# ucas-vg/PointTinyBenchmark

Measured on AMD Instinct MI355X. Metric: img/s (640x640) CPR R50-FPN fwd+loss, higher is better.
Workload: dtype fp32

## Files before the change

include/cpr_hip.h:

```cpp
#ifndef CPR_HIP_H
#define CPR_HIP_H
#ifdef __cplusplus
extern "C" {
#endif

#define CPR_ERR_ARG (-1001)
#define CPR_ERR_UNSUPPORTED (-1002)

int cpr_version(void);

#define CPR_CONV_RELU 1
#define CPR_CONV_OUT_BF16 2
#define CPR_CONV_RES_MASK 4
#define CPR_CONV_COLSUM 8
int cpr_conv2d_fwd(const float* in, const float* wgt, float* out, const float* scale, const float* bias,
                   const float* residual, const float* in_a, const float* in_b, float* gn_part, int N, int H, int W,
                   int Cin, int Cout, int KH, int KW, int stride, int pad, int Kpad, int flags, int in_relu,
                   int* variant_out, void* stream);
int cpr_conv2d_fwd_dil(const float* in, const float* wgt, float* out, const float* scale, const float* bias,
                       const float* residual, const float* in_a, const float* in_b, float* gn_part, int N, int H, int W,
                       int Cin, int Cout, int KH, int KW, int stride, int pad, int dil, int Kpad, int flags, int in_relu,
                       int* variant_out, void* stream);

int cpr_conv2d_dual_fwd(const float* in, const float* wgt, const float* in2, const float* wgt2, float* out,
                        const float* scale, const float* bias, const float* scale2, const float* bias2, int N, int H, int W,
                        int Cin, int Cout, int KH, int KW, int stride, int pad, int Kpad, int H2, int W2, int Cin2,
                        int stride2, int Kpad2, int flags, int* variant_out, void* stream);

int cpr_conv1x1_stream_fwd(const float* in, const float* wgt, float* out, const float* scale, const float* bias,
                           const float* residual, long long M, int Cin, int Cout, int flags, void* stream);

int cpr_conv_wgrad_bf16_workspace_s(int N, int H, int W, int Cin, int Cout, int k, int stride, int dy_bf16, int x_bf16);
int cpr_conv_wgrad_bf16_s(const void* dy, int dy_bf16, const void* x, int x_bf16, float* grad, void* ws, int N, int H, int W, int Cin,
                          int Cout, int k, int stride, int accumulate, void* stream);

#define CPR_WINO_IN_B8 1
#define CPR_WINO_OUT_B8 2
int cpr_wino_pack_weights(const float* wgt, float* u, int Cin, int Cout, int Kpad, void* stream);
int cpr_conv3x3_wino_fwd(const float* in, const float* u, float* out, const float* scale, const float* bias,
                         const float* in_a, const float* in_b, float* gn_part, int N, int H, int W, int Cin, int Cout,
                         int flags, int in_relu, int layout, void* stream);
int cpr_wino32_pack_weights(const float* wgt, float* u, int Cin, int Cout, int Kpad, void* stream);
int cpr_conv3x3_wino32_slots(int H, int W);
int cpr_conv3x3_wino32_fwd(const float* in, const float* u, float* out, const float* scale, const float* bias,
                           const float* in_a, const float* in_b, float* gn_part, int N, int H, int W, int Cin, int Cout,
                           int flags, int in_relu, int layout, void* stream);
int cpr_gn_apply_b8(const float* x, const float* a, const float* b, float* y, int N, int H, int W, int C, int relu,
                    void* stream);

int cpr_conv2d_fwd_bf16(const void* in, const void* wgt, const void* wgt_frag, void* out, const float* scale, const float* bias,
                        const void* residual, float* gn_part, int N, int H, int W, int Cin, int Cout, int KH, int KW,
                        int stride, int pad, int Kpad, int relu, int out_fp32, int* variant_out, void* stream);
int cpr_conv2d_bf16_mask_slots(int N, int H, int W, int Cin, int Cout, int KH, int KW, int stride, int pad, int out_fp32);
int cpr_conv2d_dgrad_bf16_fused(const void* in, const void* wgt, const void* wgt_frag, float* out32, void* out16, const float* add32,
                                const void* mask, float* part, int N, int H, int W, int Cin, int Cout, int KH, int KW, int stride,
                                int pad, int Kpad, int* variant_out, void* stream);
int cpr_stem7x7s2_bf16(const float* in, const void* wgt, const float* scale, const float* bias, void* out, int N, int H, int W,
                       int relu, int layout, void* stream);
int cpr_stem7x7s2_pool_bf16(const float* in, const void* wgt, const float* scale, const float* bias, void* out, int N, int H,
                            int W, int layout, void* stream);
int cpr_maxpool3x3s2_bf16(const void* in, void* out, int N, int H, int W, int C, void* stream);
int cpr_gn_stats_bf16(const void* x, float* part, int N, int HW, int C, int P, void* stream);
int cpr_gn_apply_bf16(const void* x, const float* a, const float* b, const void* up, void* y, int N, int H, int W,
                      int C, int UH, int UW, int relu, void* stream);

int cpr_nchw_to_nhwc4(const float* in, float* out, int N, int C, int H, int W, void* stream);
int cpr_nhwc_to_nchw(const float* in, float* out, int N, int C, int H, int W, void* stream);
int cpr_stem7x7s2_pool_f32(const float* in, const float* wgt, const float* scale, const float* bias, float* out, int N, int H,
                           int W, int layout, void* stream);
int cpr_maxpool3x3s2(const float* in, float* out, int N, int H, int W, int C, void* stream);
int cpr_stem_deep_fwd(const float* in, const float* w1, const float* s1, const float* b1, const float* w2, const float* s2,
                      const float* b2, const float* w3, const float* s3, const float* b3, float* mid1, float* mid2, void* out, int N,
                      int H, int W, int layout, int out_bf16, void* stream);
int cpr_stem3x3s2_fwd(const float* in, const float* w, const float* scale, const float* bias, float* out, int N, int H, int W,
                      int layout, void* stream);
int cpr_stem3x3s2_wgrad_workspace(int N, int H, int W);
int cpr_stem3x3s2_wgrad(const float* dy, const float* in, float* gw, float* ws, int N, int H, int W, int layout, void* stream);
int cpr_avgpool_fwd(const void* in, void* out, int N, int H, int W, int C, int s, int bf16, void* stream);
int cpr_avgpool_bwd(const void* g, const void* add, void* dx, int N, int H, int W, int C, int s, int bf16, void* stream);
int cpr_maxpool3x3s2_rec(const float* in, float* out, unsigned char* arg, int N, int H, int W, int C, void* stream);
int cpr_maxpool3x3s2_bf16_rec(const void* in, void* out, unsigned char* arg, int N, int H, int W, int C, void* stream);
int cpr_stem7x7s2_pool_f32_rec(const float* in, const float* wgt, const float* scale, const float* bias, float* out,
                               unsigned char* arg, int N, int H, int W, int layout, void* stream);
int cpr_stem7x7s2_pool_bf16_rec(const float* in, const void* wgt, const float* scale, const float* bias, void* out,
                                unsigned char* arg, int N, int H, int W, int layout, void* stream);
int cpr_stem_pool_bwd_blocks(long long M);
int cpr_stem_pool_bwd(const float* dp, const unsigned char* arg, float* dy, float* part, int N, int OH, int OW, void* stream);
int cpr_stem_wgrad_f32_workspace(int N, int H, int W);
int cpr_stem_wgrad_f32(const float* dy, const float* in, float* gw, float* ws, int N, int H, int W, int layout, void* stream);

int cpr_gn_stats(const float* x, float* part, int N, int HW, int C, int P, void* stream);
int cpr_gn_finalize(const float* part, const float* gamma, const float* beta, float* a_out, float* b_out,
                    float* mean_out, float* rstd_out, int N, int P, int C, int G, int HW, float eps, void* stream);
int cpr_gn_apply(const float* x, const float* a, const float* b, const float* up, float* y, int N, int H, int W,
                 int C, int UH, int UW, int relu, void* stream);

int cpr_box_centers(const float* boxes, float* centers, int n, void* stream);

#define CPR_PROB_SIGMOID 0
#define CPR_PROB_SOFTMAX 1
#define CPR_PROB_NORMED_SIGMOID 2
#define CPR_PROB_IDENTITY 3

int cpr_logit_project(const float* x, const float* w, const float* bias, const float* in_a, const float* in_b,
                      float* out, int N, int HW, int Cin, int J, int in_relu, void* stream);

int cpr_neg_mask_loss(const float* logit, int J, const float* centers, const int* labels, const int* gt_start,
                      const int* pad_hw, unsigned char* mask, double* partial, int N, int H, int W, int C,
                      float stride, float d2_thr, float eps, int class_wise, int prob_type, float norm_p,
                      int mask_classes, int* n_partial, void* stream);

int cpr_bag_sample(const float* map, int J, const float* centers, const int* gt_img, const int* pad_hw,
                   const float* offsets, float* pts, unsigned char* valid, float* out, int G, int K, int H, int W,
                   float stride, int align_corners, const float* pad_value, void* stream);

int cpr_grid_bag(const float* map, int J, const float* points, const int* gt_img, int R, int Kmax, float radius_px,
                 const float* pad_value, float* pts, unsigned char* valid, int* ws_cell, int* count, float* out, int G,
                 int H, int W, float stride, int align_corners, void* stream);

int cpr_mil_loss(const float* logits, int J, int ins_off, const unsigned char* valid, const int* labels,
                 const float* gt_weight, float* bag_ws, const double* neg_partial, int n_partial, int num_bags,
                 int bag_stride, int bag_off, int bag_len, int ctr_off, int ctr_stride, int ctr_count, int ctr_mod,
                 int C, float eps, int prob_type, float norm_p, int binary_ins, int allpos, float w_mil, float w_gt,
                 float w_neg, int neg_from_gt, float* out5, void* stream);

int cpr_refine(const float* logits, int J, const float* pts, const unsigned char* valid, const float* centers, int Rv,
               int ctr_stride, const int* labels, const int* gt_img, const int* gt_start, const int* img_hw,
               const unsigned char* not_refine_in, float* refine_pts, float* scores, unsigned char* not_refine,
               unsigned char* chosen, int G, int Kt, int Kv, int C, int prob_type, float norm_p, float gt_alpha,
               float merge_th, float refine_th, int use_nearest, int use_classify, int score_max, void* stream);

int cpr_point_assign(const float* points, const float* gt_bboxes, int n, int k, float scale, int pos_num,
                     long long* gt_inds, float* ws_best, int* ws_lvl, void* stream);

int cpr_hungarian_cost(const float* pred, int pred_stride, const float* logits, int C, const float* gt,
                       const int* labels, float* costT, int M, int G, float w_cls, float alpha, float gamma,
                       float eps, float w_dis, float fx, float fy, int p_norm, void* stream);
int cpr_match_cost(const float* pred, int pdim, const float* logits, int C, const float* gt, const int* labels, float* costT,
                   int M, int G, const float* terms, int ncls, int nreg, void* stream);

int cpr_lsa_topk(const float* costT, const int* m_of, const int* g_of, const long long* cost_off,
                 const long long* col_off, const long long* row_off, int num_problems, int topk, long long* gt_inds,
                 double* ws_v, double* ws_spc, int* ws_path, int* ws_row4col, unsigned char* ws_sc,
                 unsigned char* ws_active, int* ws_cols, int* ws_remaining, int* ws_pos, double* ws_u,
                 int* ws_col4row, unsigned char* ws_sr, int* status, int max_cols, int max_rows, void* stream);

int cpr_topk_desc(const float* scores, int n, int k, float* out_vals, long long* out_idx, void* stream);

int cpr_nms_candidates(const float* boxes, int box_stride, const float* scores, const float* factors, int n, int C,
                       float score_thr, float* cand_boxes, float* cand_scores, int* cand_labels, long long* cand_inds,
                       int* count, void* stream);
int cpr_nms_workspace(int n);
int cpr_nms(const float* boxes, const float* scores, const int* labels, int n, float iou_thr, long long* keep_idx,
            int* num_keep, int* ws_order, float* ws_boxes, unsigned long long* ws_mask, void* stream);
int cpr_topk_desc_batched(const float* scores, int B, int n, int k, float* out_vals, long long* out_idx, void* stream);
int cpr_nms_candidates_batched(const float* boxes, int box_stride, const float* scores, const float* factors, int B, int n,
                               int C, float score_thr, float* cand_boxes, float* cand_scores, int* cand_labels,
                               long long* cand_inds, int* count, void* stream);
int cpr_nms_batched(const float* boxes, const float* scores, const int* labels, const int* n_dev, int B, int cap,
                    float iou_thr, long long* keep_idx, int* num_keep, int* ws_order, float* ws_boxes,
                    unsigned long long* ws_mask, long long ws_stride, void* stream);

int cpr_p2p_decode(const float* reg, const float* point_anchor, float* pred, float* anchor, int N, int H, int W, int k,
                   float stride, float gamma, void* stream);
int cpr_tap_sum3x3(const float* R, const float* bias, float* out, int N, int H, int W, int J, void* stream);
int cpr_rowmax_sigmoid(const float* logits, float* out, long long M, int C, void* stream);
int cpr_sigmoid(const float* x, float* y, long long n, void* stream);
int cpr_p2p_loss(const float* logits, const float* pred, const long long* gt_inds, const float* gt_pts,
                 const int* gt_labels, const int* gt_start, double* ws_partial, float* out, int B, int M, int C,
                 float alpha, float gamma, float beta, float pos_w, float neg_w, float reg_norm, float w_cls,
                 float w_reg, int cls_mode, int reg_mode, void* stream);

int cpr_conv2d_wgrad_workspace(int N, int OH, int OW, int Cin, int Cout, int KH, int KW);
int cpr_conv2d_wgrad(const float* dy, const float* x, const float* in_a, const float* in_b, float* grad_w, float* ws,
                     int N, int H, int W, int Cin, int Cout, int KH, int KW, int stride, int pad, int in_relu,
                     int accumulate, void* stream);
int cpr_conv2d_wgrad_dil(const float* dy, const float* x, float* grad_w, float* ws, int N, int H, int W, int Cin, int Cout, int KH,
                         int KW, int stride, int pad, int dil, int accumulate, void* stream);
int cpr_conv3x3_wino_wgrad_workspace(int N, int H, int W, int Cin, int Cout);
int cpr_conv3x3_wino_wgrad(const float* dy, const float* x, const float* in_a, const float* in_b, float* grad_w, float* ws,
                           int N, int H, int W, int Cin, int Cout, int in_relu, int accumulate, void* stream);
int cpr_gn_bwd(const float* x, const float* dz, const float* a, const float* b, const float* mean, const float* rstd,
               const float* gamma, float* dx, float* dgamma, float* dbeta, float* ws_part, float* ws_k, int N, int HW,
               int C, int G, int P, int relu, int accumulate, void* stream);
int cpr_gn_bwd_bf16(const void* x_bf16, const float* dz, const float* a, const float* b, const float* mean, const float* rstd,
                    const float* gamma, float* dx, void* dx_bf16, float* dgamma, float* dbeta, float* ws_part, float* ws_k, int N,
                    int HW, int C, int G, int P, int relu, int accumulate, void* stream);
int cpr_gn_bwd_bf16_dz16(const void* x_bf16, const void* dz_bf16, const float* a, const float* b, const float* mean, const float* rstd,
                         const float* gamma, float* dx, void* dx_bf16, float* dgamma, float* dbeta, float* ws_part, float* ws_k,
                         int N, int HW, int C, int G, int P, int relu, int accumulate, void* stream);
int cpr_upsample_add_bwd(const float* dfine, float* dcoarse, int N, int H, int W, int UH, int UW, int C, int accumulate,
                         void* stream);
int cpr_relu_bwd_colsum_ws(long long M, int C);
int cpr_relu_bwd_colsum(const float* dy, const float* add, const void* y, int y_bf16, float* g_out, void* g16_out, float* colsum,
                        float* ws_part, long long M, int C, int accumulate, void* stream);
int cpr_part_colsum(const float* part, float* out, float* ws, int tiles, int C, void* stream);
int cpr_bn_fold_bwd(float* Gw, const float* weight, const float* scale, const float* mean, const float* inv_sigma,
                    const float* colsum_g, float* dgamma, float* dbeta, int Cout, int K, void* stream);
int cpr_bn_fold_bwd_part(float* Gw, const float* weight, const float* scale, const float* mean, const float* inv_sigma, const float* part,
                         int tiles, float* dgamma, float* dbeta, int Cout, int K, void* stream);
int cpr_axpby(float* y, const float* x, float alpha, float beta, long long n, void* stream);
int cpr_phase_scatter_add(const float* src, float* dst, int N, int Hs, int Ws, int C, int H, int W, int py, int px,
                          int sh, int sw, int s, void* stream);
int cpr_zero_insert(const float* dy, float* out, int N, int OH, int OW, int C, int H, int W, int s, void* stream);
int cpr_pack_weights_grouped(const float* w, const float* scale, float* out, int C, int cg, int transpose, void* stream);
int cpr_pack_weights_grouped_multi(const void* jobs_dev, int n, int total_blocks, void* stream);
int cpr_conv_group_fwd(const float* x, const float* wp, float* out, const float* scale, const float* bias, int N, int H, int W, int C,
                       int cg, int stride, int flags, void* stream);
int cpr_conv_group_wgrad_workspace(int N, int OH, int OW, int C, int cg);
int cpr_conv_group_wgrad(const float* dy, const float* x, float* grad_w, float* ws, int N, int H, int W, int C, int cg, int stride,
                         int accumulate, void* stream);
int cpr_conv_group_fwd_pitch(const float* x, const float* wp, float* out, const float* scale, const float* bias, int N, int H, int W,
                             int C, int Cp, int cg, int stride, int flags, void* stream);
int cpr_conv_group_wgrad_pitch(const float* dy, const float* x, float* grad_w, float* ws, int N, int H, int W, int C, int Cp, int cg,
                               int stride, int accumulate, void* stream);
int cpr_conv_group_fwd_dil(const float* x, const float* wp, float* out, const float* scale, const float* bias, int N, int H, int W,
                           int C, int cg, int dil, int flags, void* stream);
int cpr_conv_group_wgrad_dil(const float* dy, const float* x, float* grad_w, float* ws, int N, int H, int W, int C, int cg, int dil,
                             int accumulate, void* stream);
int cpr_res2_pack_weights(const float* w, const float* scale, float* out, int width, int transpose, void* stream);
int cpr_res2_conv_fwd(const float* x, int x_pitch, int x_off, const float* add, int add_pitch, int add_off, const float* wp, float* out,
                      int out_pitch, int out_off, const float* scale, const float* bias, int N, int IH, int IW, int OH, int OW, int width,
                      int stride, int transposed, int flags, void* stream);
int cpr_res2_conv_wgrad_workspace(int N, int OH, int OW, int width);
int cpr_res2_conv_wgrad(const float* dy, int dy_pitch, int dy_off, const float* x, int x_pitch, int x_off, const float* add, int add_pitch,
                        int add_off, float* grad_w, float* ws, int N, int H, int W, int width, int stride, int accumulate, void* stream);
int cpr_res2_relu_bwd_colsum(float* g, int g_pitch, int g_off, const float* carry, int c_pitch, int c_off, const float* y, int y_pitch,
                             int y_off, float* colsum, float* ws, long long M, int width, void* stream);
int cpr_res2_pool_fwd(const float* x, int x_pitch, int x_off, float* out, int out_pitch, int out_off, int N, int H, int W, int width,
                      int stride, void* stream);
int cpr_res2_pool_bwd(const float* dy, int dy_pitch, int dy_off, float* dx, int dx_pitch, int dx_off, int N, int H, int W, int width,
                      int stride, void* stream);
int cpr_splat_chunks(int H, int W, int w);
int cpr_splat_gap(const float* u, float* g, float* ws, int N, int H, int W, int w, void* stream);
int cpr_splat_attn(const float* g, const float* fc1w, const float* fc1b, const float* s1, const float* t1, const float* fc2w,
                   const float* fc2b, float* att, float* z, int N, int w, int inter, void* stream);
int cpr_splat_apply(const float* u, const float* att, float* out, int N, int H, int W, int w, int pool, void* stream);
int cpr_splat_attn_grad(const float* dout, const float* u, float* datt, float* ws, int N, int H, int W, int w, int pool, void* stream);
int cpr_splat_attn_bwd(const float* att, const float* datt, const float* z, const float* g, const float* fc1w, const float* fc1b,
                       const float* s1, const float* mean, const float* inv_sigma, const float* fc2w, float* dg, float* ws, float* gfc1w,
                       float* gfc1b, float* gbnw, float* gbnb, float* gfc2w, float* gfc2b, int N, int w, int inter, void* stream);
int cpr_splat_apply_bwd(const float* dout, const float* u, const float* att, const float* dg, float* du, float* colsum, float* ws, int N,
                        int H, int W, int w, int pool, void* stream);
#define CPR_DW_IN_CLAMP6 1
#define CPR_DW_RELU6 2
int cpr_dw3x3_pack(const float* w, const float* scale, float* wp, int C, void* stream);
int cpr_dw3x3_fwd(const float* x, const float* wp, const float* scale, const float* bias, float* y, int N, int H, int W, int C, int stride,
                  int flags, void* stream);
int cpr_dw3x3_dgrad_workspace(int N, int H, int W, int C);
int cpr_dw3x3_dgrad(const float* dy, const float* wp, const float* add, const float* mask, float* dx, float* colsum, float* ws, int N, int H,
                    int W, int C, int stride, void* stream);
int cpr_dw3x3_wgrad_workspace(int N, int H, int W, int C, int stride);
int cpr_dw3x3_wgrad(const float* dy, const float* x, float* grad_w, float* ws, int N, int H, int W, int C, int stride, int in_clamp6,
                    int accumulate, void* stream);
int cpr_relu6_bwd_colsum_ws(long long M, int C);
int cpr_relu6_bwd_colsum(const float* dy, const float* add, const float* y, float* g_out, float* colsum, float* ws, long long M, int C,
                         void* stream);
int cpr_clamp6(float* x, long long n, void* stream);
int cpr_subsample2(const void* x, int x_bf16, const float* a, const float* b, void* out, int N, int H, int W, int C, void* stream);
int cpr_subsample2_bwd_add(const float* dfine, const float* dcoarse, float* out, int N, int H, int W, int C, void* stream);
int cpr_relu_mask_add(const float* dz, const float* d, const void* y, int y_bf16, float* out, long long n, void* stream);
int cpr_gn_apply2(const float* x1, const float* a1, const float* b1, const float* x2, const float* a2, const float* b2, float* y, int N, int H,
                  int W, int C, void* stream);
int cpr_gn_apply2_bf16(const void* x1, const float* a1, const float* b1, const void* x2, const float* a2, const float* b2, void* y, int N,
                       int H, int W, int C, void* stream);
typedef struct cpr_bfp_level {
    const void* x;
    const float* a;
    const float* b;
    void* y;
    void* arg;
    int H, W;
    float sy, sx;
} cpr_bfp_level;
int cpr_bfp_gather(const cpr_bfp_level* levels, int L, int refine_level, float* bsf, int N, int C, int arg_wide, void* stream);
int cpr_bfp_gather_bf16(const cpr_bfp_level* levels, int L, int refine_level, void* bsf, int N, int C, int arg_wide, void* stream);
int cpr_bfp_scatter(const cpr_bfp_level* levels, int L, int refine_level, const float* ref, const float* ref_a, const float* ref_b, int N,
                    int C, int arg_wide, void* stream);
int cpr_bfp_scatter_bf16(const cpr_bfp_level* levels, int L, int refine_level, const void* ref, const float* ref_a, const float* ref_b,
                         int N, int C, int arg_wide, void* stream);
int cpr_bfp_scatter_bwd(const cpr_bfp_level* levels, int L, int refine_level, float* d_ref, int N, int C, int arg_wide, void* stream);
int cpr_bfp_gather_bwd(const cpr_bfp_level* levels, int L, int refine_level, const float* d_bsf, int N, int C, int arg_wide, void* stream);
typedef struct cpr_hrfpn_level {
    void* p;
    int H, W;
} cpr_hrfpn_level;
int cpr_hrfpn_fuse(const cpr_hrfpn_level* levels, int L, const float* bias, float* out, int N, int C, void* stream);
int cpr_hrfpn_fuse_bf16(const cpr_hrfpn_level* levels, int L, const float* bias, void* out, int N, int C, void* stream);
int cpr_hrfpn_pool(const float* out, int H0, int W0, const cpr_hrfpn_level* levels, int K1, int N, int C, void* stream);
int cpr_hrfpn_pool_bf16(const void* out, int H0, int W0, const cpr_hrfpn_level* levels, int K1, int N, int C, void* stream);
int cpr_hrfpn_pool_bwd_blocks(int N, int H0, int W0);
int cpr_hrfpn_pool_bwd(const cpr_hrfpn_level* gs, int K, float* d_out, float* part, int N, int C, void* stream);
int cpr_hrfpn_fuse_bwd(const float* d_out, int H0, int W0, const cpr_hrfpn_level* dys, int L1, int N, int C, void* stream);
typedef struct cpr_hrnet_term {
    const void* p;
    int k;
} cpr_hrnet_term;
int cpr_hrnet_fuse(const cpr_hrnet_term* terms, int T, float* out, int N, int H, int W, int C, void* stream);
int cpr_hrnet_fuse_bwd_blocks(int N, int H, int W, int C, int K);
int cpr_hrnet_fuse_bwd(const float* dy, const float* y, float* g, float* const* pools, int K, float* part, int N, int H, int W, int C,
                       void* stream);
int cpr_loss_bwd(const float* lmap, const unsigned char* neg_mask, const float* out5, const float* bag_logits,
                 const unsigned char* valid, const int* labels, const float* gt_weight, const float* bag_ws,
                 const float* centers, const int* gt_img, const float* offsets, float* dbag_ws, float* dmap, float* win_ws,
                 int* win_org, int win, int N, int H, int W, int J, int Jd, int ins_off, int G, int K, int C, float stride,
                 float eps, float w_mil, float w_gt, float w_neg, const float* upstream, void* stream);
int cpr_bag_gather_bwd(const float* dsample, int J, const float* centers, const int* gt_img, const float* offsets,
                       float* win_ws, int* win_org, int win, float* dmap, int N, int H, int W, int Jd, int G, int K,
                       float stride, void* stream);
int cpr_bag_points_gather_bwd(const float* dsample, int J, const float* pts, const int* code, const int* gt_img, float* dmap,
                              float* wout_ws, float* dbias, int N, int H, int W, int Jd, int G, int Kt, float stride,
                              int align_corners, void* stream);
int cpr_loss_bwd_general(const float* lmap, const unsigned char* neg_mask, const float* out5, const float* bag_logits,
                         const unsigned char* valid, const int* labels, const float* gt_weight, const float* bag_ws, float* dbag,
                         float* dmap, int N, int H, int W, int J, int Jd, int ins_off, int num_bags, int bag_stride, int bag_off,
                         int bag_len, int ctr_off, int ctr_stride, int ctr_count, int ctr_mod, int C, float eps, int prob_type,
                         float norm_p, int binary_ins, int allpos, float w_mil, float w_gt, float w_neg, int neg_from_gt,
                         const float* upstream, void* stream);
int cpr_pack_weights(const float* w, const float* scale, float* out, int O, int I, int KH, int KW, int colsp, int Kpad,
                     int transpose, void* stream);
int cpr_pack_weights_bf16(const float* w, const float* scale, void* out, void* frag, int O, int I, int KH, int KW, int transpose,
                          void* stream);
int cpr_spin(long long ticks, void* stream);
int cpr_bn_fold(const float* gamma, const float* beta, const float* mean, const float* var, float eps, float* scale,
                float* shift, float* inv_sigma, int C, void* stream);
int cpr_bn_train_ws(long long M, int C);
int cpr_bn_batch_stats(const float* y, const float* gamma, const float* beta, float* running_mean, float* running_var,
                       long long* num_batches_tracked, float momentum, float eps, float* mean, float* rstd, float* scale, float* shift,
                       float* center, float* cmean, float* cshift, float* ws, long long M, int C, void* stream);
int cpr_bn_apply(const float* y, const float* center, const float* scale, const float* shift, const float* residual, const float* y2,
                 const float* center2, const float* scale2, const float* shift2, float* out, long long M, int C, int relu, void* stream);
int cpr_bn_train_bwd(const float* dout, const float* z, const float* y, const float* center, const float* mean, const float* rstd,
                     const float* gamma, float* dy, float* dgamma, float* dbeta, float* ws, long long M, int C, void* stream);
int cpr_bn_sync_ws(long long M, int C);
int cpr_bn_sync_stats_local(const float* y, double* record, float* ws, long long M, int C, void* stream);
int cpr_bn_sync_stats_merge(const double* records, int R, const float* y, const float* gamma, const float* beta, float* running_mean,
                            float* running_var, long long* num_batches_tracked, float momentum, float eps, float* mean, float* rstd,
                            float* scale, float* shift, float* center, float* cmean, float* cshift, double* count, int C, void* stream);
int cpr_bn_sync_bwd_local(const float* dout, const float* z, const float* y, const float* center, const float* mean, const float* rstd,
                          float* dgamma, float* dbeta, double* record, float* ws, long long M, int C, void* stream);
// ... 74 lines not shown
```

pointtinybenchmark_amd/csrc/common.h:

```cpp
#pragma once
#include <hip/hip_runtime.h>
#include <stdint.h>

#define CPR_OK 0
#define CPR_ERR_ARG (-1001)
#define CPR_ERR_UNSUPPORTED (-1002)

#define CPR_CONV_RELU 1
#define CPR_CONV_OUT_BF16 2
#define CPR_CONV_RES_MASK 4
#define CPR_CONV_COLSUM 8

#define CPR_WINO_IN_B8 1
#define CPR_WINO_OUT_B8 2

#define CPR_CHECK_ARG(cond) \
    do {                    \
        if (!(cond)) return CPR_ERR_ARG; \
    } while (0)

#define CPR_LAUNCH_STATUS()                          \
    do {                                             \
        hipError_t e_ = hipGetLastError();           \
        return e_ == hipSuccess ? CPR_OK : -(int)e_; \
    } while (0)

typedef float f32x4 __attribute__((ext_vector_type(4)));
typedef float f32x16 __attribute__((ext_vector_type(16)));

__device__ __forceinline__ float wave_sum(float v) {
#pragma unroll
    for (int o = 32; o > 0; o >>= 1) v += __shfl_xor(v, o, 64);
    return v;
}
__device__ __forceinline__ double wave_sum_d(double v) {
#pragma unroll
    for (int o = 32; o > 0; o >>= 1) v += __shfl_xor(v, o, 64);
    return v;
}
__device__ __forceinline__ float wave_max(float v) {
#pragma unroll
    for (int o = 32; o > 0; o >>= 1) v = fmaxf(v, __shfl_xor(v, o, 64));
    return v;
}
__device__ __forceinline__ float wave_min(float v) {
#pragma unroll
    for (int o = 32; o > 0; o >>= 1) v = fminf(v, __shfl_xor(v, o, 64));
    return v;
}

__device__ __forceinline__ float sleef_expf_u10(float d) {
    const float q = rintf(__fmul_rn(d, 1.442695040888963407359924681001892137426645954152985934135449406931f));
    float s = __fmaf_rn(q, -0.693145751953125f, d);
    s = __fmaf_rn(q, -1.428606765330187045e-06f, s);
    float u = 0.000198527617612853646278381f;
    u = __fmaf_rn(u, s, 0.00139304355252534151077271f);
    u = __fmaf_rn(u, s, 0.00833336077630519866943359f);
    u = __fmaf_rn(u, s, 0.0416664853692054748535156f);
    u = __fmaf_rn(u, s, 0.166666671633720397949219f);
    u = __fmaf_rn(u, s, 0.5f);
    u = __fadd_rn(1.0f, __fmaf_rn(__fmul_rn(s, s), u, s));
    const int qi = (int)q, h = qi >> 1;
    u = __fmul_rn(u, __int_as_float((h + 127) << 23));
    u = __fmul_rn(u, __int_as_float((qi - h + 127) << 23));
    if (d < -104.f) u = 0.f;
    if (d > 104.f) u = INFINITY;
    return u;
}
__device__ __forceinline__ float sigmoid_torch_cpu(float x) { return __fdiv_rn(1.f, __fadd_rn(1.f, sleef_expf_u10(-x))); }

__device__ __forceinline__ float sq_norm(float x, float y) {
    return __fadd_rn(__fmul_rn(x, x), __fmul_rn(y, y));
}
__device__ __forceinline__ float d2_chain(float px, float py, float pn, float cx, float cy, float cn) {
    float acc = __fmul_rn(-2.f * px, cx);
    acc = __fmaf_rn(-2.f * py, cy, acc);
    acc = __fadd_rn(pn, acc);
    acc = __fadd_rn(acc, cn);
    return acc;
}

static inline int cdiv(int a, int b) { return (a + b - 1) / b; }
static inline int cpr_images_per_launch(int N, long long bytes_per_image, int align = 1) {
    const long long lim = (1ll << 31) - 1;
    if (bytes_per_image <= 0 || bytes_per_image > lim) return 0;
    const long long fit = lim / bytes_per_image;
    if (fit >= N) return N;
    const long long launches = (N + fit - 1) / fit;
    long long n = (N + launches - 1) / launches;
    n = (n + align - 1) / align * align;
    if (n > fit) n = fit / align * align;
    return (int)n;
}
static inline long long cpr_max2(long long a, long long b) { return a > b ? a : b; }
static inline long long cdivll(long long a, long long b) { return (a + b - 1) / b; }
```

pointtinybenchmark_amd/csrc/conv_wino.hip:

```cpp
#include <type_traits>
#include "common.h"

typedef float f32x2 __attribute__((ext_vector_type(2)));
typedef int i32x4 __attribute__((ext_vector_type(4)));
typedef float f32x2 __attribute__((ext_vector_type(2)));

__device__ __forceinline__ f32x2 pk_add(f32x2 a, f32x2 b) {
    f32x2 r; asm("v_pk_add_f32 %0, %1, %2" : "=v"(r) : "v"(a), "v"(b)); return r;
}
__device__ __forceinline__ f32x2 pk_sub(f32x2 a, f32x2 b) {
    f32x2 r; asm("v_pk_add_f32 %0, %1, %2 neg_lo:[0,1] neg_hi:[0,1]" : "=v"(r) : "v"(a), "v"(b)); return r;
}
__device__ __forceinline__ f32x2 pk_col01(f32x2 t01, f32x2 t23) {
    f32x2 r; asm("v_pk_add_f32 %0, %1, %2 op_sel:[0,0] op_sel_hi:[1,0] neg_lo:[0,1] neg_hi:[0,0]" : "=v"(r) : "v"(t01), "v"(t23)); return r;
}
__device__ __forceinline__ f32x2 pk_col23(f32x2 t01, f32x2 t23) {
    f32x2 r; asm("v_pk_add_f32 %0, %1, %2 op_sel:[1,0] op_sel_hi:[1,1] neg_lo:[1,0] neg_hi:[0,1]" : "=v"(r) : "v"(t01), "v"(t23)); return r;
}
__device__ __forceinline__ f32x2 pk_fma(f32x2 a, f32x2 b, f32x2 c) {
    f32x2 r; asm("v_pk_fma_f32 %0, %1, %2, %3" : "=v"(r) : "v"(a), "v"(b), "v"(c)); return r;
}

struct WinoParams {
    const float* in;
    const float* u;
    float* out;
    const float* scale;
    const float* bias;
    float* gn_part;
    const float* in_a;
    const float* in_b;
    int in_relu, out_b8;
    int N, H, W, Cin, Cout, relu, RY, RX, regions, tilesN, nch;
    int tpx;
};

constexpr int WBUF = 16 * 64 * 8;

__global__ void wino_pack_kernel(const float* __restrict__ w, float* __restrict__ u, int Cin, int Cout, int Kpad) {
    const int idx = blockIdx.x * blockDim.x + threadIdx.x;
    if (idx >= Cin * Cout) return;
    const int ci = idx % Cin, co = idx / Cin;
    float g[3][3];
#pragma unroll
    for (int a = 0; a < 3; ++a)
#pragma unroll
        for (int b = 0; b < 3; ++b) g[a][b] = w[(size_t)co * Kpad + (a * 3 + b) * Cin + ci];
    float t[4][3];
#pragma unroll
    for (int b = 0; b < 3; ++b) {
        t[0][b] = g[0][b];
        t[1][b] = 0.5f * (g[0][b] + g[1][b] + g[2][b]);
        t[2][b] = 0.5f * (g[0][b] - g[1][b] + g[2][b]);
        t[3][b] = g[2][b];
    }
    const int tn = co >> 6, cl = co & 63, chunk = ci >> 3, k = ci & 7, nch = Cin >> 3;
    float* dst = u + ((size_t)(tn * nch + chunk) * 16) * 512 + cl * 8 + 4 * ((k >> 2) ^ ((cl >> 3) & 1)) + (k & 3);
#pragma unroll
    for (int i = 0; i < 4; ++i) {
        dst[(i * 4 + 0) * 512] = t[i][0];
        dst[(i * 4 + 1) * 512] = 0.5f * (t[i][0] + t[i][1] + t[i][2]);
        dst[(i * 4 + 2) * 512] = 0.5f * (t[i][0] - t[i][1] + t[i][2]);
        dst[(i * 4 + 3) * 512] = t[i][2];
    }
}

template <int ABL, bool INB8, bool XF, int TSPREAD = 1, int VAR = 0>
__global__ __launch_bounds__(512, 1) void conv_wino_kernel(WinoParams p) {
    constexpr bool DEEP = (VAR & 1) != 0, UDMA = (VAR & 4) != 0, USINGLE = (VAR & 2) != 0 && !UDMA;
    constexpr int XFMAX = 512;
    constexpr int RAWROW = 148;
    constexpr int RAWBUF = 18 * RAWROW;
    __shared__ __attribute__((aligned(16))) float smem[4 * WBUF + 2 * RAWBUF + (XF ? 4 * XFMAX : 0)];
    float* Vs = smem;
    float* Us = smem + 2 * WBUF;

    const int tid = threadIdx.x, lane = tid & 63;
    const int wave = __builtin_amdgcn_readfirstlane(tid >> 6);
    const int wi = wave & 3;
    const int nh = wave >> 2;

    const int pixbytes = INB8 ? 32 : p.Cin * 4;
    const int chunk_bytes = INB8 ? p.H * p.W * 32 : 32;
    const __amdgpu_buffer_rsrc_t rs_in = __builtin_amdgcn_make_buffer_rsrc(
        const_cast<float*>(p.in), 0, (int)((size_t)p.N * p.H * p.W * p.Cin * 4), 0x00020000);
    const __amdgpu_buffer_rsrc_t rs_u = __builtin_amdgcn_make_buffer_rsrc(
        const_cast<float*>(p.u), 0, (int)((size_t)p.tilesN * p.nch * WBUF * 4), 0x00020000);
    float* Rw = smem + 4 * WBUF;
    float* ABs = smem + 4 * WBUF + 2 * RAWBUF;
    int par = 0;
    int upyx[2], raw_wr[2];
#pragma unroll
    for (int k = 0; k < 2; ++k) {
        const int pix = (tid + 512 * k) >> 1;
        const int py = pix / 18, px = pix - py * 18;
        upyx[k] = py << 8 | px;
        raw_wr[k] = py * RAWROW + px * 8 + (tid & 1) * 4;
    }
    const bool second_unit = wave < 3;
    const bool unit1_live = tid + 512 < 648;
    const int lch = tid & 7, tyl = (tid >> 3) & 7, ltile = wave * 8 + tyl;
    const float* t_rd = Rw + (2 * tyl) * RAWROW + (2 * wave) * 8 + lch;
    const int v_wr = ltile * 8 + 4 * ((lch >> 2) ^ ((ltile >> 3) & 1)) + (lch & 3);
    const int last = p.nch - 1;
    const float relu_floor = (XF && p.in_relu) ? 0.f : -INFINITY;

    struct Tile {
        int rg, tn, n, oy0, ox0, n0;
        int voffA[2];
        unsigned uok;
        bool any_pad, valid;
    };
    const int T = p.regions * p.tilesN;
    const int per = (T + 7) >> 3;
    const int ngrp = p.tpx > 0 ? p.tilesN / p.tpx : 1;
    const int per_r = p.tpx > 0 ? (p.regions * ngrp + 7) / 8 : 0;
    auto setup = [&](int vb) {
        Tile t;
        if (p.tpx > 0) {
            const int x = vb & 7, s = vb >> 3;
            const int sr = s / p.tpx;
            t.rg = (x / ngrp) * per_r + sr;
            t.tn = (x % ngrp) * p.tpx + (s - sr * p.tpx);
            t.valid = sr < per_r && t.rg < p.regions;
            if (!t.valid) { t.rg = 0; t.tn = 0; }
        } else {
            const int tile = (vb & 7) * per + (vb >> 3);
            t.valid = vb < per * 8 && tile < T;
            const int tl = t.valid ? tile : 0;
            t.rg = tl / p.tilesN; t.tn = tl - t.rg * p.tilesN;
        }
        t.n = t.rg / (p.RY * p.RX);
        const int rrem = t.rg - t.n * p.RY * p.RX;
        const int ry = rrem / p.RX, rx = rrem - ry * p.RX;
        t.oy0 = ry * 16; t.ox0 = rx * 16; t.n0 = t.tn * 64;
        const int img_base = INB8 ? (t.n * (p.Cin >> 3)) * p.H * p.W * 32 : t.n * p.H * p.W * p.Cin * 4;
        t.uok = 0;
#pragma unroll
        for (int k = 0; k < 2; ++k) {
            const int iy = t.oy0 - 1 + (upyx[k] >> 8), ix = t.ox0 - 1 + (upyx[k] & 255);
            const bool ok = (k == 0 || unit1_live) & ((unsigned)iy < (unsigned)p.H) & ((unsigned)ix < (unsigned)p.W);
            t.uok |= (ok ? 1u : 0u) << k;
            t.voffA[k] = ok ? img_base + (iy * p.W + ix) * pixbytes + (tid & 1) * 16 : (int)0x80000000;
        }
        t.any_pad = XF && __builtin_amdgcn_ballot_w64(t.uok != (unit1_live ? 3u : 1u)) != 0;
        return t;
    };

    f32x4 sp[2][2];
    f32x4 su[(USINGLE || UDMA) ? 1 : 2][4];
    float tab_a = 0.f, tab_b = 0.f;
    f32x2 d[4][2];
    if (ABL & 9) { sp[0][0] = f32x4{1.f, 1.f, 1.f, 1.f}; sp[0][1] = sp[0][0]; sp[1][0] = sp[0][0]; sp[1][1] = sp[0][0]; }
    Tile cur = setup(blockIdx.x);
    auto ld_a = [&](const Tile& t, int ck, int k) {
        return __builtin_bit_cast(f32x4, __builtin_amdgcn_raw_buffer_load_b128(rs_in, t.voffA[k], ck * chunk_bytes, 0));
    };
    auto ld_u = [&](const Tile& t, int ck, int z) {
        return __builtin_bit_cast(
            f32x4, __builtin_amdgcn_raw_buffer_load_b128(rs_u, tid * 16 + z * 8192, (t.tn * p.nch + ck) * (WBUF * 4), 0));
    };
    auto prefetch = [&](const Tile& t) {
        if (!(ABL & 8)) {
            sp[0][0] = ld_a(t, 0, 0); sp[1][0] = ld_a(t, 1, 0);
            if (second_unit) { sp[0][1] = ld_a(t, 0, 1); sp[1][1] = ld_a(t, 1, 1); }
        }
        if (!UDMA) {
#pragma unroll
            for (int z = 0; z < 4; ++z) { su[0][z] = ld_u(t, 0, z); if (!USINGLE) su[USINGLE ? 0 : 1][z] = ld_u(t, 1, z); }
        }
        if (XF) {
            if (tid < p.Cin) { tab_a = p.in_a[t.n * p.Cin + tid]; tab_b = p.in_b[t.n * p.Cin + tid]; }
        }
    };
    auto g_a = [&](auto set_c, int chunk, int k) {
        constexpr int SET = decltype(set_c)::value;
        if (ABL & 8) return;
        const int ck = chunk < last ? chunk : last;
        if (k == 0 || second_unit) sp[SET][k] = ld_a(cur, ck, k);
    };
    auto g_u = [&](auto set_c, int chunk, int z) {
        constexpr int SET = (USINGLE || UDMA) ? 0 : decltype(set_c)::value;
        if (!UDMA) su[SET][z] = ld_u(cur, chunk < last ? chunk : last, z);
    };
    const int lds_u0 = (int)(unsigned)(size_t)(smem + 2 * WBUF);
    const size_t u_addr = (size_t)p.u;
    const i32x4 rs_u_raw = {(int)(unsigned)u_addr, (int)(unsigned)(u_addr >> 32) & 0xffff,
                            (int)((size_t)p.tilesN * p.nch * WBUF * 4), 0x00020000};
    auto dma_u = [&](int chunk, int buf, int z) {
        const int soff = (cur.tn * p.nch + chunk) * (WBUF * 4);
        const int m0v = lds_u0 + buf * (WBUF * 4) + z * 8192 + wave * 1024;
        asm volatile("s_nop 4\n\ts_mov_b32 m0, %0\n\ts_nop 0\n\tbuffer_load_dwordx4 %1, %2, %3 offen offset:0 lds"
                     :: "s"(m0v), "v"(tid * 16 + z * 8192), "s"(rs_u_raw), "s"(soff) : "memory");
    };
    auto dma_wait = [&](auto npatch_c) {
        constexpr int NP = decltype(npatch_c)::value;
        if (NP == 0) asm volatile("s_waitcnt vmcnt(0)" ::: "memory");
        else if (second_unit) asm volatile("s_waitcnt vmcnt(%0)" :: "n"(2 * NP) : "memory");
        else asm volatile("s_waitcnt vmcnt(%0)" :: "n"(NP) : "memory");
    };
    auto affine = [&](f32x4 v, f32x4 a4, f32x4 b4, int k) {
        if (ABL & 64) v = v * a4 + b4;
        else {
            const f32x2 lo = pk_fma(f32x2{v.x, v.y}, f32x2{a4.x, a4.y}, f32x2{b4.x, b4.y});
            const f32x2 hi = pk_fma(f32x2{v.z, v.w}, f32x2{a4.z, a4.w}, f32x2{b4.z, b4.w});
            v = f32x4{lo.x, lo.y, hi.x, hi.y};
        }
        v.x = fmaxf(v.x, relu_floor); v.y = fmaxf(v.y, relu_floor); v.z = fmaxf(v.z, relu_floor); v.w = fmaxf(v.w, relu_floor);
        if (cur.any_pad) {
            asm volatile("");
            if (!((cur.uok >> k) & 1u)) v = f32x4{0.f, 0.f, 0.f, 0.f};
        }
        return v;
    };
    f32x4 xa4, xb4;
    auto xf_fetch = [&](int chunk) {
        const float* tab = ABs + par * 2 * XFMAX + (chunk < last ? chunk : last) * 8 + (tid & 1) * 4;
        xa4 = *reinterpret_cast<const f32x4*>(tab);
        xb4 = *reinterpret_cast<const f32x4*>(tab + XFMAX);
    };
    auto r_a = [&](auto set_c, int buf, int k) {
        constexpr int SET = decltype(set_c)::value;
        if (k == 1 && !second_unit) return;
        f32x4 v = sp[SET][k];
        if (XF) v = affine(v, xa4, xb4, k);
        if (k == 0 || unit1_live) *reinterpret_cast<f32x4*>(Rw + buf * RAWBUF + raw_wr[k]) = v;
    };
    auto r_a_pro = [&](int chunk01, int k) {
        if (k == 1 && !second_unit) return;
        f32x4 v = chunk01 ? sp[1][k] : sp[0][k];
        if (XF) {
            const float* tab = ABs + par * 2 * XFMAX + chunk01 * 8 + (tid & 1) * 4;
            v = affine(v, *reinterpret_cast<const f32x4*>(tab), *reinterpret_cast<const f32x4*>(tab + XFMAX), k);
        }
        if (k == 0 || unit1_live) *reinterpret_cast<f32x4*>(Rw + chunk01 * RAWBUF + raw_wr[k]) = v;
    };
    auto r_u = [&](auto set_c, int buf, int z) {
        constexpr int SET = (USINGLE || UDMA) ? 0 : decltype(set_c)::value;
        if (!UDMA) *reinterpret_cast<f32x4*>(Us + buf * WBUF + tid * 4 + z * 2048) = su[SET][z];
    };
    auto t_read = [&](int buf, int r) {
#pragma unroll
        for (int s = 0; s < 2; ++s)
            d[r][s] = f32x2{t_rd[buf * RAWBUF + r * RAWROW + (2 * s) * 8], t_rd[buf * RAWBUF + r * RAWROW + (2 * s + 1) * 8]};
    };
    auto t_row = [&](int buf, int i) {
        float* dst = Vs + buf * WBUF + (i * 4) * 512 + v_wr;
        if (ABL & 64) {
            float ts[4];
#pragma unroll
            for (int s = 0; s < 4; ++s) {
                const float d0 = d[0][s >> 1][s & 1], d1 = d[1][s >> 1][s & 1], d2 = d[2][s >> 1][s & 1], d3 = d[3][s >> 1][s & 1];
                ts[s] = i == 0 ? d0 - d2 : i == 1 ? d1 + d2 : i == 2 ? d2 - d1 : d1 - d3;
            }
            dst[0 * 512] = ts[0] - ts[2];
            dst[1 * 512] = ts[1] + ts[2];
            dst[2 * 512] = ts[2] - ts[1];
            dst[3 * 512] = ts[1] - ts[3];
            return;
        }
        f32x2 t[2];
#pragma unroll
        for (int s = 0; s < 2; ++s)
            t[s] = i == 0 ? pk_sub(d[0][s], d[2][s]) : i == 1 ? pk_add(d[1][s], d[2][s]) : i == 2 ? pk_sub(d[2][s], d[1][s])
                                                                                                  : pk_sub(d[1][s], d[3][s]);
        const f32x2 o01 = pk_col01(t[0], t[1]), o23 = pk_col23(t[0], t[1]);
        dst[0 * 512] = o01.x;
        dst[1 * 512] = o01.y;
        dst[2 * 512] = o23.x;
        dst[3 * 512] = o23.y;
    };
    const int l31 = lane & 31, half = lane >> 5;
    const float* a_lds = Vs + (wi * 4 * 64 + l31) * 8 + 4 * (half ^ ((l31 >> 3) & 1));
    const float* b_lds = Us + (wi * 4 * 64 + nh * 32 + l31) * 8 + 4 * (half ^ ((l31 >> 3) & 1));
    using Set0 = std::integral_constant<int, 0>;
    using Set1 = std::integral_constant<int, 1>;

    if (cur.valid) prefetch(cur);
    if (XF) {
        if (tid < p.Cin) { ABs[tid] = tab_a; ABs[XFMAX + tid] = tab_b; }
        __syncthreads();
    }
    for (int vb = blockIdx.x; cur.valid; vb += gridDim.x) {
    const int rg = cur.rg, n = cur.n, oy0 = cur.oy0, ox0 = cur.ox0, n0 = cur.n0;

    f32x16 acc[4][2];
#pragma unroll
    for (int j = 0; j < 4; ++j)
#pragma unroll
        for (int tb = 0; tb < 2; ++tb)
#pragma unroll
            for (int r = 0; r < 16; ++r) acc[j][tb][r] = 0.f;

    f32x4 fa0[2], fb0, fa1[2], fb1;
#define WFRAG(FA, FB, buf, j, z)                                                                                    \
    do {                                                                                                            \
        if ((z) < 2) FA[(z) < 2 ? (z) : 0] = *reinterpret_cast<const f32x4*>(a_lds + (buf) * WBUF + (j) * 512 + ((z) < 2 ? (z) : 0) * 256); \
        else FB = *reinterpret_cast<const f32x4*>(b_lds + (buf) * WBUF + (j) * 512);                                \
    } while (0)
#define WMFMA(FA, FB, j, q) \
    acc[j][(q) & 1] = __builtin_amdgcn_mfma_f32_32x32x2f32(FA[(q) & 1][(q) >> 1], FB[(q) >> 1], acc[j][(q) & 1], 0, 0, 0)
    r_a_pro(0, 0); r_a_pro(0, 1);
    r_a_pro(1, 0); r_a_pro(1, 1);
    if (UDMA) {
#pragma unroll
        for (int z = 0; z < 4; ++z) dma_u(0, 0, z);
#pragma unroll
        for (int z = 0; z < 4; ++z) dma_u(1, 1, z);
    }
#pragma unroll
    for (int z = 0; z < 4; ++z) r_u(Set0{}, 0, z);
    g_a(Set0{}, 2, 0); g_a(Set0{}, 2, 1);
    if (DEEP) { g_a(Set1{}, 3, 0); g_a(Set1{}, 3, 1); }
#pragma unroll
    for (int z = 0; z < 4; ++z) g_u(Set0{}, USINGLE ? 1 : 2, z);
    __syncthreads();
#pragma unroll
    for (int r = 0; r < 4; ++r) t_read(0, r);
#pragma unroll
    for (int i = 0; i < 4; ++i) t_row(0, i);
    if (TSPREAD == 1) {
#pragma unroll
        for (int r = 0; r < 4; ++r) t_read(1, r);
    }
    if (UDMA) dma_wait(std::integral_constant<int, DEEP ? 2 : 1>{});
    __syncthreads();
#pragma unroll
    for (int z = 0; z < 3; ++z) WFRAG(fa0, fb0, 0, 0, z);

    auto iteration = [&](auto nxt_c, int c) {
        const int buf = c & 1;
        const std::integral_constant<int, DEEP ? 1 - decltype(nxt_c)::value : 0> pset_c{};
#pragma unroll
        for (int q = 0; q < 8; ++q) {
            WMFMA(fa0, fb0, 0, q);
            if (q < 3 && !(ABL & 2)) WFRAG(fa1, fb1, buf, 1, q);
            if (!(ABL & 1)) {
                if (TSPREAD == 0 || TSPREAD == 2) { if (q >= 4) t_read(buf ^ 1, q - 4); }
                else { if (q == 3) t_row(buf ^ 1, 0); if (q == 6) t_row(buf ^ 1, 1); }
            }
            __builtin_amdgcn_sched_barrier(0);
        }
#pragma unroll
        for (int q = 0; q < 8; ++q) {
            WMFMA(fa1, fb1, 1, q);
            if (q < 3 && !(ABL & 2)) WFRAG(fa0, fb0, buf, 2, q);
            if (!(ABL & 1)) {
                if (q & 1) r_u(nxt_c, buf ^ 1, q >> 1);
                else if (TSPREAD == 0) t_row(buf ^ 1, q >> 1);
                else if (TSPREAD == 2) {
                    if (q == 0) {
#pragma unroll
                        for (int i = 0; i < 4; ++i) t_row(buf ^ 1, i);
                    }
                }
                else if (q == 2) t_row(buf ^ 1, 2);
                else if (q == 6) t_row(buf ^ 1, 3);
                if (XF && q == 7) xf_fetch(c + 2);
            }
            __builtin_amdgcn_sched_barrier(0);
        }
#pragma unroll
        for (int q = 0; q < 8; ++q) {
            WMFMA(fa0, fb0, 2, q);
            if (q < 3 && !(ABL & 2)) WFRAG(fa1, fb1, buf, 3, q);
            if (!(ABL & 1)) {
                if (q == 3) { r_a(pset_c, buf, 0); if (TSPREAD == 2) r_a(pset_c, buf, 1); }
                if (q == 4 && TSPREAD != 2) r_a(pset_c, buf, 1);
                if (q == 5 || q == 6 || q == 7) g_u(nxt_c, c + (USINGLE ? 2 : 3), q - 5);
            }
            __builtin_amdgcn_sched_barrier(0);
        }
        asm volatile("" ::: "memory");
        if (UDMA) dma_wait(std::integral_constant<int, DEEP ? 1 : 0>{});
        __builtin_amdgcn_s_waitcnt(0xc07f);
        if (!(ABL & 4)) __builtin_amdgcn_s_barrier();
        asm volatile("" ::: "memory");
        __builtin_amdgcn_sched_barrier(0);
#pragma unroll
        for (int q = 0; q < 8; ++q) {
            WMFMA(fa1, fb1, 3, q);
            if (q < 3 && !(ABL & 2)) WFRAG(fa0, fb0, buf ^ 1, 0, q);
            if (!(ABL & 1)) {
                if (UDMA) {
                    if (q < 4 && c + 2 < p.nch) dma_u(c + 2, buf, q);
                    if (q == 4) g_a(pset_c, c + (DEEP ? 4 : 3), 0);
                    if (q == 6) g_a(pset_c, c + (DEEP ? 4 : 3), 1);
                } else {
                    if (q == 3) g_a(pset_c, c + (DEEP ? 4 : 3), 0);
                    if (q == 5) g_a(pset_c, c + (DEEP ? 4 : 3), 1);
                    if (q == 7) g_u(nxt_c, c + (USINGLE ? 2 : 3), 3);
                }
                if (TSPREAD == 1 && q >= 4) t_read(buf, q - 4);
            }
            __builtin_amdgcn_sched_barrier(0);
        }
    };
    for (int c = 0; c < p.nch; c += 2) {
        iteration(Set1{}, c);
        iteration(Set0{}, c + 1);
    }
#undef WFRAG
#undef WMFMA

    if (ABL & 32) {
        asm volatile("" ::"v"(acc[0][0]), "v"(acc[0][1]), "v"(acc[1][0]), "v"(acc[1][1]));
        asm volatile("" ::"v"(acc[2][0]), "v"(acc[2][1]), "v"(acc[3][0]), "v"(acc[3][1]));
        cur = setup(vb + gridDim.x);
        if (cur.valid) prefetch(cur);
        if (XF && tid < p.Cin) { ABs[(par ^ 1) * 2 * XFMAX + tid] = tab_a; ABs[(par ^ 1) * 2 * XFMAX + XFMAX + tid] = tab_b; }
        par ^= 1;
        __syncthreads();
        continue;
    }
    const Tile nxt = setup(vb + gridDim.x);
    if (nxt.valid) prefetch(nxt);
    __syncthreads();
    float* Rs = smem;
#pragma unroll
    for (int tb = 0; tb < 2; ++tb)
#pragma unroll
        for (int r = 0; r < 16; ++r) {
            const int trow = tb * 32 + (r & 3) + 8 * (r >> 2) + 4 * half;
            const float m0 = acc[0][tb][r], m1 = acc[1][tb][r], m2 = acc[2][tb][r], m3 = acc[3][tb][r];
            Rs[((wi * 2 + 0) * 64 + trow) * 64 + nh * 32 + l31] = m0 + m1 + m2;
            Rs[((wi * 2 + 1) * 64 + trow) * 64 + nh * 32 + l31] = m1 - m2 - m3;
        }
    __syncthreads();
    const int c4 = tid & 15;
    const int co = n0 + c4 * 4;
    f32x4 sc = {1.f, 1.f, 1.f, 1.f}, bi = {0.f, 0.f, 0.f, 0.f};
    if (p.scale) sc = *reinterpret_cast<const f32x4*>(p.scale + co);
    if (p.bias) bi = *reinterpret_cast<const f32x4*>(p.bias + co);
    const __amdgpu_buffer_rsrc_t rs_out = __builtin_amdgcn_make_buffer_rsrc(
        p.out, 0, (int)((size_t)p.N * p.H * p.W * p.Cout * 4), 0x00020000);
    f32x4 gs = {0.f, 0.f, 0.f, 0.f}, gq = {0.f, 0.f, 0.f, 0.f};
#pragma unroll
    for (int k = 0; k < 2; ++k) {
        const int t = (tid >> 4) + 32 * k;
        const int oy = oy0 + 2 * (t & 7), ox = ox0 + 2 * (t >> 3);
#pragma unroll
        for (int b = 0; b < 2; ++b) {
            const f32x4 r0 = *reinterpret_cast<const f32x4*>(Rs + ((0 * 2 + b) * 64 + t) * 64 + c4 * 4);
            const f32x4 r1 = *reinterpret_cast<const f32x4*>(Rs + ((1 * 2 + b) * 64 + t) * 64 + c4 * 4);
            const f32x4 r2 = *reinterpret_cast<const f32x4*>(Rs + ((2 * 2 + b) * 64 + t) * 64 + c4 * 4);
            const f32x4 r3 = *reinterpret_cast<const f32x4*>(Rs + ((3 * 2 + b) * 64 + t) * 64 + c4 * 4);
            f32x4 y[2] = {r0 + r1 + r2, r1 - r2 - r3};
#pragma unroll
            for (int a = 0; a < 2; ++a) {
                f32x4 v = y[a] * sc + bi;
                if (p.relu) { v.x = fmaxf(v.x, 0.f); v.y = fmaxf(v.y, 0.f); v.z = fmaxf(v.z, 0.f); v.w = fmaxf(v.w, 0.f); }
                const bool ok = (oy + a < p.H) & (ox + b < p.W);
                const unsigned off = !ok ? 0x80000000u
                    : p.out_b8 ? (unsigned)((((n * (p.Cout >> 3) + (co >> 3)) * p.H + oy + a) * p.W + ox + b) * 8 + (co & 7)) * 4u
                               : (unsigned)(((n * p.H + oy + a) * p.W + ox + b) * p.Cout + co) * 4u;
                if (!(ABL & 16)) __builtin_amdgcn_raw_buffer_store_b128(__builtin_bit_cast(__attribute__((ext_vector_type(4))) unsigned, v), rs_out, (int)off, 0, 0);
                if (p.gn_part && ok) { gs += v; gq += v * v; }
            }
        }
    }
    if (p.gn_part) {
#pragma unroll
        for (int e = 0; e < 4; ++e) {
            gs[e] += __shfl_xor(gs[e], 16, 64); gs[e] += __shfl_xor(gs[e], 32, 64);
            gq[e] += __shfl_xor(gq[e], 16, 64); gq[e] += __shfl_xor(gq[e], 32, 64);
        }
        __syncthreads();
        if (lane < 16) {
#pragma unroll
            for (int e = 0; e < 4; ++e) {
                smem[(wave * 64 + c4 * 4 + e) * 2 + 0] = gs[e];
                smem[(wave * 64 + c4 * 4 + e) * 2 + 1] = gq[e];
            }
        }
        __syncthreads();
        if (tid < 64) {
            float s = 0.f, q = 0.f;
#pragma unroll
            for (int w8 = 0; w8 < 8; ++w8) { s += smem[(w8 * 64 + tid) * 2]; q += smem[(w8 * 64 + tid) * 2 + 1]; }
            float* dst = p.gn_part + ((size_t)rg * p.Cout + n0 + tid) * 2;
            dst[0] = s; dst[1] = q;
        }
    }
    if (XF && tid < p.Cin) {
        ABs[(par ^ 1) * 2 * XFMAX + tid] = tab_a;
        ABs[(par ^ 1) * 2 * XFMAX + XFMAX + tid] = tab_b;
    }
    par ^= 1;
    __syncthreads();
    cur = nxt;
    }
}

#ifdef CPR_BENCH_HOOKS
static int wino_sched = 0, wino_ablate = 0, wino_var = -1, wino_tpx = -1;
extern "C" int cpr_wino_set_variant(int sched, int ablate) {
    CPR_CHECK_ARG(sched >= 0 && sched <= 2 && ablate >= 0 && ablate <= 64);
    wino_sched = sched;
    wino_ablate = ablate;
    return CPR_OK;
}
extern "C" int cpr_wino_set_staging(int var, int tpx) {
    CPR_CHECK_ARG(var >= -1 && var <= 5 && tpx >= -1 && tpx <= 2);
    wino_var = var;
    wino_tpx = tpx;
    return CPR_OK;
}
#else
constexpr int wino_sched = 0, wino_ablate = 0, wino_var = -1, wino_tpx = -1;
#endif
constexpr int WINO_VAR_DEFAULT = 4, WINO_TPX_DEFAULT = 0;
extern "C" int cpr_wino_pack_weights(const float* wgt, float* u, int Cin, int Cout, int Kpad, hipStream_t stream) {
    CPR_CHECK_ARG(wgt && u && Cin > 0 && Cout > 0 && Cin % 8 == 0 && Cout % 64 == 0 && Kpad >= 9 * Cin);
    hipLaunchKernelGGL(wino_pack_kernel, dim3(cdiv(Cin * Cout, 256)), dim3(256), 0, stream, wgt, u, Cin, Cout, Kpad);
    CPR_LAUNCH_STATUS();
}
static int wino_fwd_launch(const float* in, const float* u, float* out, const float* scale, const float* bias,
                           const float* in_a, const float* in_b, float* gn_part, int N, int H, int W, int Cin,
                           int Cout, int flags, int in_relu, int layout, hipStream_t stream) {
    CPR_CHECK_ARG(in && u && out && N > 0 && H > 0 && W > 0);
    CPR_CHECK_ARG(Cin > 0 && Cout > 0 && Cin % 16 == 0 && Cout % 64 == 0 && Cin >= 32);
    CPR_CHECK_ARG((flags & ~CPR_CONV_RELU) == 0 && (layout & ~3) == 0);
    if (in_a) CPR_CHECK_ARG(in_b && Cin <= 512);
    if ((long long)N * H * W * Cin * 4 >= (1ll << 31) || (long long)N * H * W * Cout * 4 >= (1ll << 31)) return CPR_ERR_UNSUPPORTED;
    WinoParams p;
    p.in = in; p.u = u; p.out = out; p.scale = scale; p.bias = bias; p.gn_part = gn_part;
    p.in_a = in_a; p.in_b = in_b; p.in_relu = in_relu; p.out_b8 = (layout & CPR_WINO_OUT_B8) ? 1 : 0;
    p.N = N; p.H = H; p.W = W; p.Cin = Cin; p.Cout = Cout; p.relu = flags & CPR_CONV_RELU;
    p.RY = (H + 15) / 16; p.RX = (W + 15) / 16;
    p.regions = N * p.RY * p.RX; p.tilesN = Cout / 64; p.nch = Cin / 8;
    const long long T = (long long)p.regions * p.tilesN;
    if (T >= (1ll << 30)) return CPR_ERR_UNSUPPORTED;
    static int cu_of_device[64] = {};
    int dev = 0, ncu = 256;
    if (hipGetDevice(&dev) == hipSuccess && dev >= 0 && dev < 64) {
        if (cu_of_device[dev] == 0) {
            int v = 0;
            if (hipDeviceGetAttribute(&v, hipDeviceAttributeMultiprocessorCount, dev) == hipSuccess && v > 0) cu_of_device[dev] = v;
        }
        if (cu_of_device[dev] > 0) ncu = cu_of_device[dev];
    }
    ncu = (ncu + 7) / 8 * 8;
    int grid = (int)((T + 7) / 8 * 8);
    if (grid > ncu) grid = ncu;
    const bool b8 = (layout & CPR_WINO_IN_B8) != 0, xf = in_a != nullptr;
    p.tpx = wino_tpx >= 0 ? wino_tpx : WINO_TPX_DEFAULT;
    if (p.tpx > 0 && !(p.tilesN % p.tpx == 0 && 8 % (p.tilesN / p.tpx) == 0)) p.tpx = 0;
    if (p.tpx > 0) {
        const long long per_r = ((long long)p.regions * (p.tilesN / p.tpx) + 7) / 8;
        const long long vbs = 8 * per_r * p.tpx;
        if (vbs < grid) grid = (int)vbs;
    }
    const int var = wino_var >= 0 ? wino_var : WINO_VAR_DEFAULT;
#define WLAUNCHV(A_, F_, V_)                                                                                                      \
    do {                                                                                                                         \
        constexpr int TX_ = F_ == 2 ? 2 : 0 ^ F_, TP_ = F_ == 2 ? 2 : 1 ^ F_;                                                     \
        if (b8 && xf) hipLaunchKernelGGL((conv_wino_kernel<A_, true, true, TX_, V_>), dim3(grid), dim3(512), 0, stream, p);       \
        else if (b8) hipLaunchKernelGGL((conv_wino_kernel<A_, true, false, TP_, V_>), dim3(grid), dim3(512), 0, stream, p);       \
        else if (xf) hipLaunchKernelGGL((conv_wino_kernel<A_, false, true, TX_, V_>), dim3(grid), dim3(512), 0, stream, p);       \
        else hipLaunchKernelGGL((conv_wino_kernel<A_, false, false, TP_, V_>), dim3(grid), dim3(512), 0, stream, p);              \
    } while (0)
#define WLAUNCH(A_, F_) WLAUNCHV(A_, F_, WINO_VAR_DEFAULT)
#ifdef CPR_BENCH_HOOKS
    if ((var != WINO_VAR_DEFAULT || wino_sched == 2) && !wino_ablate) {
        switch (var * 3 + wino_sched) {
            case 0: WLAUNCHV(0, 0, 0); break;
            case 1: WLAUNCHV(0, 1, 0); break;
            case 2: WLAUNCHV(0, 2, 0); break;
            case 6: WLAUNCHV(0, 0, 2); break;
            case 7: WLAUNCHV(0, 1, 2); break;
            case 8: WLAUNCHV(0, 2, 2); break;
            case 9: WLAUNCHV(0, 0, 3); break;
            case 10: WLAUNCHV(0, 1, 3); break;
            case 11: WLAUNCHV(0, 2, 3); break;
            case 12: WLAUNCHV(0, 0, 4); break;
            case 13: WLAUNCHV(0, 1, 4); break;
            case 14: WLAUNCHV(0, 2, 4); break;
            default: return CPR_ERR_UNSUPPORTED;
        }
    } else if (wino_ablate || wino_sched) {
        switch (wino_ablate) {
            case 0: WLAUNCH(0, 1); break;
            case 1: WLAUNCH(1, 0); break;
            case 2: WLAUNCH(2, 0); break;
            case 4: WLAUNCH(4, 0); break;
            case 8: WLAUNCH(8, 0); break;
            case 16: WLAUNCH(16, 0); break;
            case 32: WLAUNCH(32, 0); break;
            case 64: WLAUNCH(64, 0); break;
            default: WLAUNCH(7, 0); break;
        }
    } else
#endif
    WLAUNCH(0, 0);
#undef WLAUNCH
#undef WLAUNCHV
    CPR_LAUNCH_STATUS();
}

extern "C" int cpr_conv3x3_wino_fwd(const float* in, const float* u, float* out, const float* scale, const float* bias,
                                    const float* in_a, const float* in_b, float* gn_part, int N, int H, int W, int Cin,
                                    int Cout, int flags, int in_relu, int layout, hipStream_t stream) {
    CPR_CHECK_ARG(N > 0 && H > 0 && W > 0 && Cin > 0 && Cout > 0);
    const int per = cpr_images_per_launch(N, (long long)H * W * cpr_max2(Cin, Cout) * 4);
    if (per <= 0) return CPR_ERR_UNSUPPORTED;
    const size_t slots = (size_t)((H + 15) / 16) * ((W + 15) / 16);
    for (int n0 = 0; n0 < N; n0 += per) {
        const int n = N - n0 < per ? N - n0 : per;
        const int rc = wino_fwd_launch(in + (size_t)n0 * H * W * Cin, u, out + (size_t)n0 * H * W * Cout, scale, bias,
                                       in_a ? in_a + (size_t)n0 * Cin : nullptr, in_b ? in_b + (size_t)n0 * Cin : nullptr,
                                       gn_part ? gn_part + (size_t)n0 * slots * Cout * 2 : nullptr, n, H, W, Cin, Cout, flags,
                                       in_relu, layout, stream);
        if (rc != CPR_OK) return rc;
    }
    return CPR_OK;
}
```

pointtinybenchmark_amd/csrc/conv_wino32.hip:

```cpp
#include "common.h"

typedef float f32x2 __attribute__((ext_vector_type(2)));
typedef int i32x4 __attribute__((ext_vector_type(4)));

struct Wino32Params {
    const float* in;
    const float* u;
    float* out;
    const float* scale;
    const float* bias;
    float* gn_part;
    const float* in_a;
    const float* in_b;
    int in_relu, in_b8, out_b8;
    int N, H, W, Cin, Cout, relu, RY, RX, regions, tilesN, nch;
    int stagger;
};

constexpr int W32_V = 16 * 32 * 4;
constexpr int W32_U = 16 * 64 * 4;
constexpr int W32_RAW = 192 * 4;
constexpr int W32_XFMAX = 256;
constexpr int W32_LDS = 2 * W32_V + 3 * W32_U + 4 * W32_RAW + 2 * W32_XFMAX;

__global__ void wino32_pack_kernel(const float* __restrict__ w, float* __restrict__ u, int Cin, int Cout, int Kpad) {
    const int idx = blockIdx.x * blockDim.x + threadIdx.x;
    if (idx >= Cin * Cout) return;
    const int ci = idx % Cin, co = idx / Cin;
    float g[3][3];
#pragma unroll
    for (int a = 0; a < 3; ++a)
#pragma unroll
        for (int b = 0; b < 3; ++b) g[a][b] = w[(size_t)co * Kpad + (a * 3 + b) * Cin + ci];
    float t[4][3];
#pragma unroll
    for (int b = 0; b < 3; ++b) {
        t[0][b] = g[0][b];
        t[1][b] = 0.5f * (g[0][b] + g[1][b] + g[2][b]);
        t[2][b] = 0.5f * (g[0][b] - g[1][b] + g[2][b]);
        t[3][b] = g[2][b];
    }
    const int tn = co >> 6, cl = co & 63, chunk = ci >> 2, k = ci & 3, nch = Cin >> 2;
    float* dst = u + ((size_t)(tn * nch + chunk) * 16) * 256 + cl * 4 + k;
#pragma unroll
    for (int i = 0; i < 4; ++i) {
        dst[(i * 4 + 0) * 256] = t[i][0];
        dst[(i * 4 + 1) * 256] = 0.5f * (t[i][0] + t[i][1] + t[i][2]);
        dst[(i * 4 + 2) * 256] = 0.5f * (t[i][0] - t[i][1] + t[i][2]);
        dst[(i * 4 + 3) * 256] = t[i][2];
    }
}

template <bool XF, int ABL = 0>
__global__ __launch_bounds__(256, 2) void conv_wino32_kernel(Wino32Params p) {
    __shared__ __attribute__((aligned(16))) float smem[W32_LDS];
    float* Vs = smem;
    float* Us = smem + 2 * W32_V;
    float* Rw = smem + 2 * W32_V + 3 * W32_U;
    float* ABs = Rw + 4 * W32_RAW;

    const int tid = threadIdx.x, lane = tid & 63;
    const int wave = __builtin_amdgcn_readfirstlane(tid >> 6);
    const int l31 = lane & 31, half = lane >> 5;

    const size_t in_addr = (size_t)p.in, u_addr = (size_t)p.u;
    const i32x4 rs_in = {(int)(unsigned)in_addr, (int)(unsigned)(in_addr >> 32) & 0xffff,
                         (int)((size_t)p.N * p.H * p.W * p.Cin * 4), 0x00020000};
    const i32x4 rs_u = {(int)(unsigned)u_addr, (int)(unsigned)(u_addr >> 32) & 0xffff,
                        (int)((size_t)p.tilesN * p.nch * W32_U * 4), 0x00020000};
    const int lds_u0 = (int)(unsigned)(size_t)Us, lds_raw0 = (int)(unsigned)(size_t)Rw;
    const int pixbytes = p.in_b8 ? 32 : p.Cin * 4;
    const int upy = tid / 18, upx = tid - upy * 18;
    const bool unit_live = tid < 180;
    const int tch = lane & 3, ttx = (lane >> 2) & 7;
    const int t_rd = (2 * wave + half) * 72 + (2 * ttx) * 4 + tch;
    const int t_wrA = ((half ? 12 : 0) * 32 + wave * 8 + ttx) * 4 + tch;
    const int t_wrB = ((half ? 8 : 4) * 32 + wave * 8 + ttx) * 4 + tch;
    const int a_rd = (wave * 4 * 32 + l31) * 4 + 2 * half;
    const int b_rd = (wave * 4 * 64 + l31) * 4 + 2 * half;

    const int T = p.regions * p.tilesN;
    const int per = (T + 7) >> 3;
    const float relu_floor = (XF && p.in_relu) ? 0.f : -INFINITY;

    if ((int)blockIdx.x >= (int)(gridDim.x >> 1)) {
        for (int s = 0; s < p.stagger; ++s) __builtin_amdgcn_s_sleep(127);
    }

    int cur_n = -1;
    for (int vb = blockIdx.x;; vb += gridDim.x) {
        const int tile = (vb & 7) * per + (vb >> 3);
        if (!(vb < per * 8 && tile < T)) break;
        const int rg = tile / p.tilesN, tn = tile - rg * p.tilesN;
        const int n = rg / (p.RY * p.RX);
        const int rrem = rg - n * p.RY * p.RX;
        const int ry = rrem / p.RX, rx = rrem - ry * p.RX;
        const int oy0 = ry * 8, ox0 = rx * 16, n0 = tn * 64;
        const int iy = oy0 - 1 + upy, ix = ox0 - 1 + upx;
        const bool uok = unit_live & ((unsigned)iy < (unsigned)p.H) & ((unsigned)ix < (unsigned)p.W);
        const int img_base = p.in_b8 ? (n * (p.Cin >> 3)) * p.H * p.W * 32 : n * p.H * p.W * p.Cin * 4;
        const int voff_a = uok ? img_base + (iy * p.W + ix) * pixbytes : (int)0x80000000;

        auto dma_u = [&](int chunk, int slot) {
            if (ABL & 2) return;
            const int ck = chunk < p.nch ? chunk : p.nch - 1;
            const int soff = (tn * p.nch + ck) * (W32_U * 4);
#pragma unroll
            for (int z = 0; z < 4; ++z) {
                const int piece = (z * 4 + wave) * 1024;
                const int m0v = lds_u0 + slot * (W32_U * 4) + piece;
                asm volatile("s_nop 4\n\ts_mov_b32 m0, %0\n\ts_nop 0\n\tbuffer_load_dwordx4 %1, %2, %3 offen offset:0 lds"
                             :: "s"(m0v), "v"(piece + lane * 16), "s"(rs_u), "s"(soff) : "memory");
            }
        };
        auto dma_a = [&](int chunk, int slot) {
            if ((ABL & 2) || wave >= 3) return;
            const int ck = chunk < p.nch ? chunk : p.nch - 1;
            const int soff = p.in_b8 ? (ck >> 1) * (p.H * p.W * 32) + (ck & 1) * 16 : ck * 16;
            const int m0v = lds_raw0 + slot * (W32_RAW * 4) + wave * 1024;
            asm volatile("s_nop 4\n\ts_mov_b32 m0, %0\n\ts_nop 0\n\tbuffer_load_dwordx4 %1, %2, %3 offen offset:0 lds"
                         :: "s"(m0v), "v"(voff_a), "s"(rs_in), "s"(soff) : "memory");
        };
        auto wait_older_than_this_chunk = [&]() {
            if (ABL & 2) return;
            if (wave < 3) asm volatile("s_waitcnt vmcnt(5)" ::: "memory");
            else asm volatile("s_waitcnt vmcnt(4)" ::: "memory");
        };
        auto affine_pass = [&](int chunk, int slot) {
            if (!XF || (ABL & 1)) return;
            if (unit_live) {
                const int ck = chunk < p.nch ? chunk : p.nch - 1;
                float* q = Rw + slot * W32_RAW + tid * 4;
                f32x4 v = *reinterpret_cast<const f32x4*>(q);
                const f32x4 a4 = *reinterpret_cast<const f32x4*>(ABs + ck * 4);
                const f32x4 b4 = *reinterpret_cast<const f32x4*>(ABs + W32_XFMAX + ck * 4);
                v = v * a4 + b4;
                v.x = fmaxf(v.x, relu_floor); v.y = fmaxf(v.y, relu_floor); v.z = fmaxf(v.z, relu_floor); v.w = fmaxf(v.w, relu_floor);
                if (!uok) v = f32x4{0.f, 0.f, 0.f, 0.f};
                *reinterpret_cast<f32x4*>(q) = v;
            }
        };
        float e[3][4] = {};
        auto t_read = [&](int slot, int r) {
            if (ABL & 1) return;
#pragma unroll
            for (int s = 0; s < 4; ++s) e[r][s] = Rw[slot * W32_RAW + t_rd + r * 72 + s * 4];
        };
        auto t_write = [&](int buf) {
            if (ABL & 1) return;
            float* dA = Vs + buf * W32_V + t_wrA;
            float* dB = Vs + buf * W32_V + t_wrB;
            float ta[4], tb[4];
#pragma unroll
            for (int s = 0; s < 4; ++s) {
                ta[s] = e[0][s] - e[2][s];
                tb[s] = e[1][s] + (half ? -e[0][s] : e[2][s]);
            }
            dA[0 * 128] = ta[0] - ta[2]; dA[1 * 128] = ta[1] + ta[2]; dA[2 * 128] = ta[2] - ta[1]; dA[3 * 128] = ta[1] - ta[3];
            dB[0 * 128] = tb[0] - tb[2]; dB[1 * 128] = tb[1] + tb[2]; dB[2 * 128] = tb[2] - tb[1]; dB[3 * 128] = tb[1] - tb[3];
        };

        if (XF && n != cur_n) {
            for (int c = tid; c < p.Cin; c += 256) { ABs[c] = p.in_a[n * p.Cin + c]; ABs[W32_XFMAX + c] = p.in_b[n * p.Cin + c]; }
            cur_n = n;
        }
        dma_u(0, 0); dma_u(1, 1);
        dma_a(0, 0); dma_a(1, 1); dma_a(2, 2); dma_a(3, 3);
        asm volatile("s_waitcnt vmcnt(0)" ::: "memory");
        __syncthreads();
        affine_pass(0, 0); affine_pass(1, 1);
        if (XF) __syncthreads();
#pragma unroll
        for (int r = 0; r < 3; ++r) t_read(0, r);
        t_write(0);
        __syncthreads();

        f32x16 acc[4][2];
#pragma unroll
        for (int j = 0; j < 4; ++j)
#pragma unroll
            for (int nb = 0; nb < 2; ++nb)
#pragma unroll
                for (int r = 0; r < 16; ++r) acc[j][nb][r] = 0.f;

        for (int c = 0; c < p.nch; ++c) {
            const int b = c & 1;
            const int uslot = c % 3;
            dma_u(c + 2, (c + 2) % 3);
            dma_a(c + 4, c & 3);
            const float* va = Vs + b * W32_V + a_rd;
            const float* ub = Us + uslot * W32_U + b_rd;
            f32x2 fa[2], fb[2][2];
            fa[0] = *reinterpret_cast<const f32x2*>(va);
            fb[0][0] = *reinterpret_cast<const f32x2*>(ub);
            fb[0][1] = *reinterpret_cast<const f32x2*>(ub + 128);
#pragma unroll
            for (int j = 0; j < 4; ++j) {
                const int cu = j & 1, nx = cu ^ 1;
                acc[j][0] = __builtin_amdgcn_mfma_f32_32x32x2f32(fa[cu].x, fb[cu][0].x, acc[j][0], 0, 0, 0);
                if (j < 3 && !(ABL & 8)) {
                    fa[nx] = *reinterpret_cast<const f32x2*>(va + (j + 1) * 128);
                    fb[nx][0] = *reinterpret_cast<const f32x2*>(ub + (j + 1) * 256);
                    fb[nx][1] = *reinterpret_cast<const f32x2*>(ub + (j + 1) * 256 + 128);
                }
                __builtin_amdgcn_sched_barrier(0);
                acc[j][1] = __builtin_amdgcn_mfma_f32_32x32x2f32(fa[cu].x, fb[cu][1].x, acc[j][1], 0, 0, 0);
                if (j == 0) { t_read((c + 1) & 3, 0); }
                if (j == 1) { t_read((c + 1) & 3, 1); }
                if (j == 2) { t_read((c + 1) & 3, 2); }
                __builtin_amdgcn_sched_barrier(0);
                acc[j][0] = __builtin_amdgcn_mfma_f32_32x32x2f32(fa[cu].y, fb[cu][0].y, acc[j][0], 0, 0, 0);
                if (j == 1) affine_pass(c + 2, (c + 2) & 3);
                __builtin_amdgcn_sched_barrier(0);
                acc[j][1] = __builtin_amdgcn_mfma_f32_32x32x2f32(fa[cu].y, fb[cu][1].y, acc[j][1], 0, 0, 0);
                if (j == 3) t_write(b ^ 1);
                __builtin_amdgcn_sched_barrier(0);
            }
            asm volatile("" ::: "memory");
            wait_older_than_this_chunk();
            __builtin_amdgcn_s_waitcnt(0xc07f);
            if (!(ABL & 4)) __builtin_amdgcn_s_barrier();
            asm volatile("" ::: "memory");
        }
        asm volatile("s_waitcnt vmcnt(0)" ::: "memory");
        __syncthreads();

        float* Rs = smem;
#pragma unroll
        for (int nb = 0; nb < 2; ++nb)
#pragma unroll
            for (int r = 0; r < 16; ++r) {
                const int trow = (r & 3) + 8 * (r >> 2) + 4 * half;
                const float m0 = acc[0][nb][r], m1 = acc[1][nb][r], m2 = acc[2][nb][r], m3 = acc[3][nb][r];
                Rs[((wave * 2 + 0) * 32 + trow) * 64 + nb * 32 + l31] = m0 + m1 + m2;
                Rs[((wave * 2 + 1) * 32 + trow) * 64 + nb * 32 + l31] = m1 - m2 - m3;
            }
        __syncthreads();
        const int c4 = tid & 15;
        const int co = n0 + c4 * 4;
        f32x4 sc = {1.f, 1.f, 1.f, 1.f}, bi = {0.f, 0.f, 0.f, 0.f};
        if (p.scale) sc = *reinterpret_cast<const f32x4*>(p.scale + co);
        if (p.bias) bi = *reinterpret_cast<const f32x4*>(p.bias + co);
        const __amdgpu_buffer_rsrc_t rs_out = __builtin_amdgcn_make_buffer_rsrc(
            p.out, 0, (int)((size_t)p.N * p.H * p.W * p.Cout * 4), 0x00020000);
        f32x4 gs = {0.f, 0.f, 0.f, 0.f}, gq = {0.f, 0.f, 0.f, 0.f};
#pragma unroll
        for (int k = 0; k < 4; ++k) {
            const int it = (tid >> 4) + 16 * k;
            const int t = it & 31, bq = it >> 5;
            const int oy = oy0 + 2 * (t >> 3), ox = ox0 + 2 * (t & 7) + bq;
            const f32x4 r0 = *reinterpret_cast<const f32x4*>(Rs + ((0 * 2 + bq) * 32 + t) * 64 + c4 * 4);
            const f32x4 r1 = *reinterpret_cast<const f32x4*>(Rs + ((1 * 2 + bq) * 32 + t) * 64 + c4 * 4);
            const f32x4 r2 = *reinterpret_cast<const f32x4*>(Rs + ((2 * 2 + bq) * 32 + t) * 64 + c4 * 4);
            const f32x4 r3 = *reinterpret_cast<const f32x4*>(Rs + ((3 * 2 + bq) * 32 + t) * 64 + c4 * 4);
            f32x4 y[2] = {r0 + r1 + r2, r1 - r2 - r3};
#pragma unroll
            for (int a = 0; a < 2; ++a) {
                f32x4 v = y[a] * sc + bi;
                if (p.relu) { v.x = fmaxf(v.x, 0.f); v.y = fmaxf(v.y, 0.f); v.z = fmaxf(v.z, 0.f); v.w = fmaxf(v.w, 0.f); }
                const bool ok = (oy + a < p.H) & (ox < p.W);
                const unsigned off = !ok ? 0x80000000u
                    : p.out_b8 ? (unsigned)((((n * (p.Cout >> 3) + (co >> 3)) * p.H + oy + a) * p.W + ox) * 8 + (co & 7)) * 4u
                               : (unsigned)(((n * p.H + oy + a) * p.W + ox) * p.Cout + co) * 4u;
                __builtin_amdgcn_raw_buffer_store_b128(__builtin_bit_cast(__attribute__((ext_vector_type(4))) unsigned, v), rs_out, (int)off, 0, 0);
                if (p.gn_part && ok) { gs += v; gq += v * v; }
            }
        }
        if (p.gn_part) {
#pragma unroll
            for (int q = 0; q < 4; ++q) {
                gs[q] += __shfl_xor(gs[q], 16, 64); gs[q] += __shfl_xor(gs[q], 32, 64);
                gq[q] += __shfl_xor(gq[q], 16, 64); gq[q] += __shfl_xor(gq[q], 32, 64);
            }
            __syncthreads();
            if (lane < 16) {
#pragma unroll
                for (int q = 0; q < 4; ++q) {
                    smem[(wave * 64 + c4 * 4 + q) * 2 + 0] = gs[q];
                    smem[(wave * 64 + c4 * 4 + q) * 2 + 1] = gq[q];
                }
            }
            __syncthreads();
            if (tid < 64) {
                float s = 0.f, q = 0.f;
#pragma unroll
                for (int w4 = 0; w4 < 4; ++w4) { s += smem[(w4 * 64 + tid) * 2]; q += smem[(w4 * 64 + tid) * 2 + 1]; }
                float* dst = p.gn_part + ((size_t)rg * p.Cout + n0 + tid) * 2;
                dst[0] = s; dst[1] = q;
            }
        }
        __syncthreads();
    }
}

#ifdef CPR_BENCH_HOOKS
static int w32_ablate = 0, w32_wg_per_cu = 2, w32_stagger_pct = 100;
extern "C" int cpr_wino32_set_debug(int ablate, int wg_per_cu, int stagger_pct) {
    CPR_CHECK_ARG(ablate >= 0 && ablate <= 15 && wg_per_cu >= 1 && wg_per_cu <= 2 && stagger_pct >= 0 && stagger_pct <= 400);
    w32_ablate = ablate; w32_wg_per_cu = wg_per_cu; w32_stagger_pct = stagger_pct;
    return CPR_OK;
}
#else
constexpr int w32_ablate = 0, w32_wg_per_cu = 2, w32_stagger_pct = 100;
#endif
extern "C" int cpr_wino32_pack_weights(const float* wgt, float* u, int Cin, int Cout, int Kpad, hipStream_t stream) {
    CPR_CHECK_ARG(wgt && u && Cin > 0 && Cout > 0 && Cin % 4 == 0 && Cout % 64 == 0 && Kpad >= 9 * Cin);
    hipLaunchKernelGGL(wino32_pack_kernel, dim3(cdiv(Cin * Cout, 256)), dim3(256), 0, stream, wgt, u, Cin, Cout, Kpad);
    CPR_LAUNCH_STATUS();
}

extern "C" int cpr_conv3x3_wino32_slots(int H, int W) { return H > 0 && W > 0 ? ((H + 7) / 8) * ((W + 15) / 16) : CPR_ERR_ARG; }

static int wino32_fwd_launch(const float* in, const float* u, float* out, const float* scale, const float* bias,
                             const float* in_a, const float* in_b, float* gn_part, int N, int H, int W, int Cin,
                             int Cout, int flags, int in_relu, int layout, hipStream_t stream) {
    CPR_CHECK_ARG(in && u && out && N > 0 && H > 0 && W > 0);
    CPR_CHECK_ARG(Cin > 0 && Cout > 0 && Cin % 8 == 0 && Cout % 64 == 0 && Cin >= 16);
    CPR_CHECK_ARG((flags & ~CPR_CONV_RELU) == 0 && (layout & ~3) == 0);
    if (in_a) CPR_CHECK_ARG(in_b && Cin <= W32_XFMAX);
    if ((long long)N * H * W * Cin * 4 >= (1ll << 31) || (long long)N * H * W * Cout * 4 >= (1ll << 31)) return CPR_ERR_UNSUPPORTED;
    Wino32Params p;
    p.in = in; p.u = u; p.out = out; p.scale = scale; p.bias = bias; p.gn_part = gn_part;
    p.in_a = in_a; p.in_b = in_b; p.in_relu = in_relu;
    p.in_b8 = (layout & CPR_WINO_IN_B8) ? 1 : 0; p.out_b8 = (layout & CPR_WINO_OUT_B8) ? 1 : 0;
    p.N = N; p.H = H; p.W = W; p.Cin = Cin; p.Cout = Cout; p.relu = flags & CPR_CONV_RELU;
    p.RY = (H + 7) / 8; p.RX = (W + 15) / 16;
    p.regions = N * p.RY * p.RX; p.tilesN = Cout / 64; p.nch = Cin / 4;
    const long long T = (long long)p.regions * p.tilesN;
    if (T >= (1ll << 30)) return CPR_ERR_UNSUPPORTED;
    static int cu_of_device[64] = {};
    int dev = 0, ncu = 256;
    if (hipGetDevice(&dev) == hipSuccess && dev >= 0 && dev < 64) {
        if (cu_of_device[dev] == 0) {
            int v = 0;
            if (hipDeviceGetAttribute(&v, hipDeviceAttributeMultiprocessorCount, dev) == hipSuccess && v > 0) cu_of_device[dev] = v;
        }
        if (cu_of_device[dev] > 0) ncu = cu_of_device[dev];
    }
    ncu = (ncu + 7) / 8 * 8;
    int grid = (int)((T + 7) / 8 * 8);
    if (grid > w32_wg_per_cu * ncu) grid = w32_wg_per_cu * ncu;
    p.stagger = grid > ncu ? (int)(((long long)p.nch * 16 * 65 * w32_stagger_pct / 100 + 8127) / 8128) : 0;
#ifdef CPR_BENCH_HOOKS
#define W32L(A_)                                                                                                      \
    do {                                                                                                              \
        if (in_a) hipLaunchKernelGGL((conv_wino32_kernel<true, A_>), dim3(grid), dim3(256), 0, stream, p);           \
        else hipLaunchKernelGGL((conv_wino32_kernel<false, A_>), dim3(grid), dim3(256), 0, stream, p);               \
    } while (0)
    switch (w32_ablate) {
        case 0: W32L(0); break;
        case 1: W32L(1); break;
        case 2: W32L(2); break;
        case 3: W32L(3); break;
        case 4: W32L(4); break;
        case 7: W32L(7); break;
        case 8: W32L(8); break;
        case 15: W32L(15); break;
        default: return CPR_ERR_UNSUPPORTED;
    }
#undef W32L
#else
    if (in_a) hipLaunchKernelGGL((conv_wino32_kernel<true>), dim3(grid), dim3(256), 0, stream, p);
    else hipLaunchKernelGGL((conv_wino32_kernel<false>), dim3(grid), dim3(256), 0, stream, p);
#endif
    CPR_LAUNCH_STATUS();
}

extern "C" int cpr_conv3x3_wino32_fwd(const float* in, const float* u, float* out, const float* scale, const float* bias,
                                      const float* in_a, const float* in_b, float* gn_part, int N, int H, int W, int Cin,
                                      int Cout, int flags, int in_relu, int layout, hipStream_t stream) {
    CPR_CHECK_ARG(N > 0 && H > 0 && W > 0 && Cin > 0 && Cout > 0);
    const int per = cpr_images_per_launch(N, (long long)H * W * cpr_max2(Cin, Cout) * 4);
    if (per <= 0) return CPR_ERR_UNSUPPORTED;
    const size_t slots = (size_t)((H + 7) / 8) * ((W + 15) / 16);
    for (int n0 = 0; n0 < N; n0 += per) {
        const int n = N - n0 < per ? N - n0 : per;
        const int rc = wino32_fwd_launch(in + (size_t)n0 * H * W * Cin, u, out + (size_t)n0 * H * W * Cout, scale, bias,
                                         in_a ? in_a + (size_t)n0 * Cin : nullptr, in_b ? in_b + (size_t)n0 * Cin : nullptr,
                                         gn_part ? gn_part + (size_t)n0 * slots * Cout * 2 : nullptr, n, H, W, Cin, Cout, flags,
                                         in_relu, layout, stream);
        if (rc != CPR_OK) return rc;
    }
    return CPR_OK;
}
```

pointtinybenchmark_amd/ops.py:

```python
import collections
import ctypes
import math

import torch

from . import _lib


def _ptr(t):
    return ctypes.c_void_p(t.data_ptr()) if t is not None else None


def _stream():
    return ctypes.c_void_p(torch.cuda.current_stream().cuda_stream)


def _check(t, dtype=torch.float32):
    if not t.is_cuda:
        raise _lib.CprHipError('HIP op called with a CPU tensor: the product path has no CPU fallback')
    ok = t.dtype in dtype if isinstance(dtype, tuple) else t.dtype == dtype
    assert ok and t.is_contiguous(), (t.dtype, t.stride())
    return t


ACT = (torch.float32, torch.bfloat16)


def as_nchw(x_nhwc):
    return x_nhwc.permute(0, 3, 1, 2)


def pad32(c):
    return (c + 31) // 32 * 32


def as_nchw_padded(buf, C):
    if buf.shape[-1] == C:
        return as_nchw(buf)
    view = buf[..., :C].permute(0, 3, 1, 2)
    view._cpr_padded = buf
    return view


def padded_buffer(x):
    buf = getattr(x, '_cpr_padded', None)
    if buf is None:
        return None
    N, C, H, W = x.shape
    ok = buf.dim() == 4 and tuple(buf.shape[:3]) == (N, H, W) and buf.shape[3] == pad32(C) and buf.is_contiguous() and \
        x.data_ptr() == buf.data_ptr() and x.stride() == (H * W * buf.shape[3], 1, W * buf.shape[3], buf.shape[3])
    return buf if ok else None


def from_nchw(x):
    y = x.permute(0, 2, 3, 1)
    if y.is_contiguous():
        return y
    return nchw_to_nhwc(x)


NECK_INPUT_COPIES = [0]


def neck_input(x):
    C = x.shape[1]
    if C % 32 == 0 or C <= 4:
        return from_nchw(x)
    buf = padded_buffer(x)
    if buf is None:
        N, _, H, W = x.shape
        buf = torch.zeros((N, H, W, pad32(C)), device=x.device, dtype=torch.float32)
        buf[..., :C].copy_(x.permute(0, 2, 3, 1))
        NECK_INPUT_COPIES[0] += 1
    return buf


def nchw_to_nhwc(x):
    N, C, H, W = x.shape
    if C <= 4:
        x = _check(x.contiguous())
        out = torch.empty((N, H, W, 4), device=x.device, dtype=torch.float32)
        _lib.call('cpr_nchw_to_nhwc4', _ptr(x), _ptr(out), N, C, H, W, _stream())
        return out
    return x.permute(0, 2, 3, 1).contiguous()


def nhwc_to_nchw_dense(x_nhwc):
    N, H, W, C = x_nhwc.shape
    out = torch.empty((N, C, H, W), device=x_nhwc.device, dtype=torch.float32)
    _lib.call('cpr_nhwc_to_nchw', _ptr(_check(x_nhwc)), _ptr(out), N, C, H, W, _stream())
    return out


class PackedConv:
    wfrag = None
    wino = None
    wino32 = None
    ready = None
    groups = 1
    cg = None
    C = None
    dilation = 1

    def _packed(self):
        self.ready = record_ready()

    def __init__(self, weight, stride=1, padding=0, dtype=torch.float32, groups=1, pitch=None, dilation=1):
        dilation = int(dilation)
        assert dilation >= 1, 'dilation must be >= 1, got %d' % dilation
        if dilation != 1 and dtype == torch.bfloat16:
            raise NotImplementedError('dilation=%d: a dilated convolution runs in the fp32 compute mode only (the bf16 kernels have no '
                                      'dilated form)' % dilation)
        if groups > 1:
            self._init_grouped(weight, stride, padding, dtype, groups, None, 0, pitch, dilation)
            return
        assert pitch is None, 'a channel pitch is the grouped kernels\' (dense layers pad their packs)'
        Cout, Cin, KH, KW = weight.shape
        if dilation != 1:
            assert (KH, KW) == (3, 3) and stride == 1 and padding == dilation and Cin % 32 == 0, \
                'dilation=%d: 3x3 / stride 1 / padding == dilation with Cin %% 32 == 0, got weight %s stride %d padding %d' \
                % (dilation, tuple(weight.shape), stride, padding)
            self.dilation = dilation
        w = weight.detach().to(torch.float32).permute(0, 2, 3, 1)
        self.dtype = dtype
        if dtype == torch.bfloat16:
            assert Cin % 64 == 0, 'bf16 conv needs Cin % 64 == 0'
            self.Cout, self.Cin, self.KH, self.KW, self.Kpad = Cout, Cin, KH, KW, KH * KW * Cin
            self.stride, self.padding = stride, padding
            if weight.is_cuda:
                self._pack_bf16(weight, None, 0)
                return
            self.w = w.reshape(Cout, KH * KW * Cin).to(torch.bfloat16).contiguous()
            return
        if Cin <= 4:
            cin_p = 4
        else:
            assert Cin % 32 == 0, 'input channels must be a multiple of 32 (or <= 4 for the stem)'
            cin_p = Cin
        K = KH * KW * cin_p
        Kpad = (K + 31) // 32 * 32
        self.Cout, self.Cin, self.KH, self.KW, self.Kpad = Cout, cin_p, KH, KW, Kpad
        self.stride, self.padding = stride, padding
        if weight.is_cuda:
            src = weight.detach()
            if src.dtype != torch.float32 or not src.is_contiguous():
                src = src.float().contiguous()
            self.w = torch.empty((Cout, Kpad), device=weight.device, dtype=torch.float32)
            _lib.call('cpr_pack_weights', _ptr(src), None, _ptr(self.w), Cout, Cin, KH, KW, cin_p, Kpad, 0, _stream())
            self._packed()
            return
        wp = torch.zeros((Cout, KH, KW, cin_p), device=weight.device, dtype=torch.float32)
        wp[..., :Cin] = w
        packed = torch.zeros((Cout, Kpad), device=weight.device, dtype=torch.float32)
        packed[:, :K] = wp.reshape(Cout, K)
        self.w = packed.contiguous()

    def _init_grouped(self, weight, stride, padding, dtype, groups, scale, transpose, pitch=None, dilation=1):
        C, cg, KH, KW = weight.shape
        pitch = C if pitch is None else int(pitch)
        assert pitch >= C and pitch % 4 == 0, 'grouped conv: the channel pitch %d must be a multiple of 4 and >= C = %d' % (pitch, C)
        if dtype != torch.float32:
            raise NotImplementedError('a grouped convolution (groups=%d) runs in the fp32 compute mode only, not in %s' % (groups, dtype))
        assert weight.is_cuda, 'the grouped pack is built on the device'
        assert cg * groups == C and cg in GROUP_WIDTHS and (KH, KW) == (3, 3) and padding == dilation and stride in (1, 2), \
            'grouped conv: 3x3 / padding == dilation / stride 1 or 2 with a group width in %s, got weight %s groups %d stride %d ' \
            'padding %d dilation %d' % (GROUP_WIDTHS, tuple(weight.shape), groups, stride, padding, dilation)
        assert dilation == 1 or (stride == 1 and pitch == C), \
            'grouped conv: dilation=%d needs stride 1 and unpitched maps, got stride %d pitch %d (C = %d)' % (dilation, stride, pitch, C)
        self.dtype, self.groups, self.cg, self.C = torch.float32, groups, cg, C
        self.Cout, self.Cin, self.KH, self.KW, self.Kpad = pitch, pitch, 3, 3, 9 * cg
        self.stride, self.padding = stride, dilation
        if dilation != 1:
            self.dilation = dilation
        src = weight.detach()
        if src.dtype != torch.float32 or not src.is_contiguous():
            src = src.float().contiguous()
        self.w = torch.empty((9 * cg * C,), device=weight.device, dtype=torch.float32)
        _lib.call('cpr_pack_weights_grouped', _ptr(src), _ptr(scale), _ptr(self.w), C, cg, int(transpose), _stream())
        self._packed()

    @staticmethod
    def dgrad_padding(k, padding, dilation=1):
        return dilation * (k - 1) - padding

    @classmethod
    def for_dgrad_grouped(cls, weight, groups, scale=None, pitch=None, dilation=1):
        self = cls.__new__(cls)
        self._init_grouped(weight, 1, self.dgrad_padding(3, dilation, dilation), torch.float32, groups, scale, 1, pitch, dilation)
        return self

    def _pack_bf16(self, weight, scale, transpose):
        src = weight.detach()
        if src.dtype != torch.float32 or not src.is_contiguous():
            src = src.float().contiguous()
        O, I, KH, KW = src.shape
        rows = self.Cout
        self.w = torch.empty((rows, self.Kpad), device=src.device, dtype=torch.bfloat16)
        want_frag = rows % 256 == 0 and self.Kpad % 64 == 0 and WFRAG[0]
        if want_frag:
            self.wfrag = torch.empty((rows // 64, self.Kpad // 16, 2, 2, 32, 8), device=src.device, dtype=torch.bfloat16)
        _lib.call('cpr_pack_weights_bf16', _ptr(src), _ptr(scale), _ptr(self.w), _ptr(self.wfrag if want_frag else None), O, I, KH, KW,
                  int(transpose), _stream())
        self._packed()

    @classmethod
    def for_dgrad_bf16(cls, weight, padding, scale=None, pad_override=None):
        Cout, Cin, KH, KW = weight.shape
        assert (KH == KW or pad_override is not None) and weight.is_cuda and Cout % 64 == 0
        self = cls.__new__(cls)
        self.dtype = torch.bfloat16
        self.Cout, self.Cin, self.KH, self.KW, self.Kpad = Cin, Cout, KH, KW, KH * KW * Cout
        self.stride, self.padding = 1, (KH - 1 - padding if pad_override is None else pad_override)
        self._pack_bf16(weight, scale, 1)
        return self

    def frag_image(self):
        if self.dtype != torch.bfloat16 or self.Cout % 256 != 0 or self.Kpad % 64 != 0 or not WFRAG[0]:
            return None
        if self.wfrag is None:
            G, KS = self.Cout // 64, self.Kpad // 16
            self.wfrag = self.w.view(G, 32, 2, KS, 2, 8).permute(0, 3, 2, 4, 1, 5).contiguous()
            self._packed()
        return self.wfrag

    @classmethod
    def for_dgrad(cls, weight, padding, scale=None, pad_override=None, dilation=1):
        Cout, Cin, KH, KW = weight.shape
        assert (KH == KW or pad_override is not None) and weight.is_cuda
        dilation = int(dilation)
        assert dilation == 1 or ((KH, KW) == (3, 3) and pad_override is None and padding == dilation and Cout % 32 == 0), \
            'dilation=%d: the data gradient of a 3x3 / padding == dilation layer, got weight %s padding %d' \
            % (dilation, tuple(weight.shape), padding)
        assert Cout % 32 == 0 or Cout <= 4, 'gradient channels must be a multiple of 32 (or <= 4)'
        self = cls.__new__(cls)
        self.dtype = torch.float32
        cols_p = 4 if Cout <= 4 else Cout
        K = KH * KW * cols_p
        Kpad = (K + 31) // 32 * 32
        self.Cout, self.Cin, self.KH, self.KW, self.Kpad = Cin, cols_p, KH, KW, Kpad
        self.stride, self.padding = 1, (self.dgrad_padding(KH, padding, dilation) if pad_override is None else pad_override)
        if dilation != 1:
            self.dilation = dilation
        src = weight.detach()
        if src.dtype != torch.float32 or not src.is_contiguous():
            src = src.float().contiguous()
        self.w = torch.empty((Cin, Kpad), device=weight.device, dtype=torch.float32)
        _lib.call('cpr_pack_weights', _ptr(src), _ptr(scale), _ptr(self.w), Cout, Cin, KH, KW, cols_p, Kpad, 1, _stream())
        self._packed()
        return self

    def out_hw(self, H, W):
        d = self.dilation
        return ((H + 2 * self.padding - d * (self.KH - 1) - 1) // self.stride + 1,
                (W + 2 * self.padding - d * (self.KW - 1) - 1) // self.stride + 1)


CONV_RELU, CONV_OUT_BF16, CONV_RES_MASK, CONV_COLSUM = 1, 2, 4, 8
GROUP_WIDTHS = (4, 8, 16, 24, 32, 40, 48, 56)
WFRAG = [True]
TRACE_CONV_VARIANT = [False, None]

WINOGRAD = [True]
WINO_MIN_FILL = 0.6


def record_ready():
    if not torch.cuda.is_available() or torch.cuda.is_current_stream_capturing():
        return None
    ev = torch.cuda.Event()
    ev.record()
    return ev, torch.cuda.current_stream().cuda_stream


def wait_ready(ready):
    if ready is None or torch.cuda.is_current_stream_capturing():
        return ready
    ev, stream = ready
    if ev.query():
        return None
    cur = torch.cuda.current_stream()
    if cur.cuda_stream != stream:
        cur.wait_event(ev)
    return ready


def pack_ready(pc):
    if pc.ready is not None:
        pc.ready = wait_ready(pc.ready)


def wino_eligible(pc, H, W, dtype=torch.float32):
    if pc.dilation != 1:
        return False
    if not (pc.groups == 1 and WINOGRAD[0] and dtype == torch.float32 and pc.dtype == torch.float32 and pc.KH == 3 and pc.KW == 3 and
            pc.stride == 1 and pc.padding == 1 and pc.Cin % 16 == 0 and pc.Cin >= 32 and pc.Cout % 64 == 0):
        return False
    fill = (H * W) / float(((H + 15) // 16 * 16) * ((W + 15) // 16 * 16))
    return fill >= WINO_MIN_FILL


WINO_TILE = ['auto']


def wino_instance(pc, H, W, fused_affine):
    can32 = pc.Cin % 8 == 0 and (not fused_affine or pc.Cin <= 256)
    if WINO_TILE[0] == '64' or not can32:
        return '64'
    if WINO_TILE[0] == '32':
        return '32'
    return WINO_AUTO(pc, H, W, fused_affine)


WINO32_MAX_PIXELS = 40 * 40


def WINO_AUTO(pc, H, W, fused_affine):
    return '32' if H * W <= WINO32_MAX_PIXELS else '64'


def wino_gn_slots(pc, H, W, fused_affine):
    if wino_instance(pc, H, W, fused_affine) == '32':
        return ((H + 7) // 8) * ((W + 15) // 16)
    return ((H + 15) // 16) * ((W + 15) // 16)


def is_b8(x):
    return x.dim() == 5 and x.shape[-1] == 8


def conv3x3_wino(x, pc, scale=None, bias=None, relu=False, gn_part=False, out=None, in_ab=None, in_relu=False,
                 out_b8=False):
    _check(x, ACT)
    in_b8 = is_b8(x)
    if in_b8:
        N, _, H, W, _ = x.shape
        Cin = x.shape[1] * 8
    else:
        N, H, W, Cin = x.shape
    assert x.dtype == torch.float32 and Cin == pc.Cin and pc.KH == 3 and pc.stride == 1 and pc.padding == 1
    inst = wino_instance(pc, H, W, in_ab is not None)
    attr, pack_fn = ('wino32', 'cpr_wino32_pack_weights') if inst == '32' else ('wino', 'cpr_wino_pack_weights')
    if getattr(pc, attr) is None:
        pack_ready(pc)
        wino = torch.empty((16 * pc.Cin * pc.Cout,), device=x.device, dtype=torch.float32)
        _lib.call(pack_fn, _ptr(pc.w), _ptr(wino), pc.Cin, pc.Cout, pc.Kpad, _stream())
        setattr(pc, attr, wino)
        pc._packed()
    pack_ready(pc)
    shape = (N, pc.Cout // 8, H, W, 8) if out_b8 else (N, H, W, pc.Cout)
    if out is None:
        out = torch.empty(shape, device=x.device, dtype=torch.float32)
    assert tuple(out.shape) == shape and out.is_contiguous()
    part = None
    if gn_part:
        part = torch.empty((N * wino_gn_slots(pc, H, W, in_ab is not None), pc.Cout, 2), device=x.device, dtype=torch.float32)
    a = b = None
    if in_ab is not None:
        a, b = in_ab
        assert Cin <= 512
    _lib.call('cpr_conv3x3_wino32_fwd' if inst == '32' else 'cpr_conv3x3_wino_fwd', _ptr(x), _ptr(getattr(pc, attr)), _ptr(out),
              _ptr(scale), _ptr(bias), _ptr(a), _ptr(b), _ptr(part), N, H, W, Cin, pc.Cout, CONV_RELU if relu else 0, int(in_relu),
              (1 if in_b8 else 0) | (2 if out_b8 else 0), _stream())
    if TRACE_CONV_VARIANT[0]:
        TRACE_CONV_VARIANT[1] = ('wino32' if inst == '32' else 'wino',
                                 (1 if in_b8 else 0) | (2 if out_b8 else 0) | (4 if in_ab is not None else 0))
    return (out, part) if gn_part else out


def gn_apply_b8(x, a=None, b=None, relu=False):
    assert is_b8(x)
    N, C8, H, W, _ = _check(x, ACT).shape
    y = torch.empty((N, H, W, C8 * 8), device=x.device, dtype=torch.float32)
    _lib.call('cpr_gn_apply_b8', _ptr(x), _ptr(a), _ptr(b), _ptr(y), N, H, W, C8 * 8, int(relu), _stream())
    return y


def conv2d(x, pc, scale=None, bias=None, residual=None, relu=False, in_ab=None, in_relu=False, gn_part=False,
           out=None, out_dtype=None, res_mask=False, colsum=False, out_b8=False):
    _check(x, ACT)
    pack_ready(pc)
    if is_b8(x):
        assert residual is None and not (res_mask or colsum) and out_dtype in (None, torch.float32) and \
            wino_eligible(pc, x.shape[2], x.shape[3], x.dtype), 'channel-blocked input needs a Winograd-eligible layer'
        return conv3x3_wino(x, pc, scale, bias, relu, gn_part, out, in_ab, in_relu, out_b8)
    N, H, W, Cin = x.shape
    assert Cin == pc.Cin, (Cin, pc.Cin)
    assert x.dtype == pc.dtype, 'weights were packed for %s, input is %s' % (pc.dtype, x.dtype)
    OH, OW = pc.out_hw(H, W)
    odt = out_dtype or x.dtype
    if pc.groups > 1:
        assert residual is None and in_ab is None and not (in_relu or gn_part or res_mask or colsum or out_b8) and \
            odt == torch.float32, 'the grouped conv has no residual, GroupNorm-statistics, fused-input-affine or bf16 form'
        if out is None:
            out = torch.empty((N, OH, OW, pc.Cout), device=x.device, dtype=torch.float32)
        assert tuple(out.shape) == (N, OH, OW, pc.Cout) and out.is_contiguous()
        if scale is not None or bias is not None:
            assert (scale is None or _check(scale).numel() >= pc.C) and (bias is None or _check(bias).numel() >= pc.C)
        if pc.dilation != 1:
            assert Cin == pc.C and pc.stride == 1
            _lib.call('cpr_conv_group_fwd_dil', _ptr(x), _ptr(pc.w), _ptr(out), _ptr(scale), _ptr(bias), N, H, W, Cin, pc.cg, pc.dilation,
                      CONV_RELU if relu else 0, _stream())
        elif Cin == pc.C:
            _lib.call('cpr_conv_group_fwd', _ptr(x), _ptr(pc.w), _ptr(out), _ptr(scale), _ptr(bias), N, H, W, Cin, pc.cg, pc.stride,
                      CONV_RELU if relu else 0, _stream())
        else:
            _lib.call('cpr_conv_group_fwd_pitch', _ptr(x), _ptr(pc.w), _ptr(out), _ptr(scale), _ptr(bias), N, H, W, pc.C, Cin, pc.cg,
                      pc.stride, CONV_RELU if relu else 0, _stream())
        if TRACE_CONV_VARIANT[0]:
            TRACE_CONV_VARIANT[1] = ('group', pc.cg)
        return out
    if residual is None and not (res_mask or colsum) and odt == torch.float32 and wino_eligible(pc, H, W, x.dtype) and \
            (in_ab is None or Cin <= 512):
        return conv3x3_wino(x, pc, scale, bias, relu, gn_part, out, in_ab, in_relu, out_b8)
    assert not out_b8, 'channel-blocked output is produced by the Winograd layers only (check wino_eligible first)'
    if pc.dilation != 1:
        assert in_ab is None and not (in_relu or gn_part) and odt == torch.float32 and x.dtype == torch.float32, \
            'a dilated conv (dilation=%d) has no fused-input-affine, GroupNorm-statistics or bf16 form' % pc.dilation
        if out is None:
            out = torch.empty((N, OH, OW, pc.Cout), device=x.device, dtype=torch.float32)
        assert tuple(out.shape) == (N, OH, OW, pc.Cout) and out.is_contiguous()
        part = torch.empty(((N * OH * OW + 63) // 64, pc.Cout, 2), device=x.device, dtype=torch.float32) if colsum else None
        variant = ctypes.c_int(0) if (colsum or TRACE_CONV_VARIANT[0]) else None
        flags = (CONV_RELU if relu else 0) | (CONV_RES_MASK if res_mask else 0) | (CONV_COLSUM if colsum else 0)
        _lib.call('cpr_conv2d_fwd_dil', _ptr(x), _ptr(pc.w), _ptr(out), _ptr(scale), _ptr(bias), _ptr(residual), None, None, _ptr(part),
                  N, H, W, Cin, pc.Cout, pc.KH, pc.KW, pc.stride, pc.padding, pc.dilation, pc.Kpad, flags, 0,
                  ctypes.byref(variant) if variant is not None else None, _stream())
        if variant is not None:
            TRACE_CONV_VARIANT[1] = ('fp32_dil', variant.value)
        if colsum:
            bm = variant.value // 1000000
            return out, TilePartials(part, (N * OH * OW + bm - 1) // bm, pc.Cout)
        return out
    if out is None:
        out = torch.empty((N, OH, OW, pc.Cout), device=x.device, dtype=odt)
    part = None
    if gn_part:
        assert (OH * OW) % 128 == 0 and not colsum
        part = torch.empty((N * OH * OW // 128, pc.Cout, 2), device=x.device, dtype=torch.float32)
    if colsum and x.dtype != torch.bfloat16:
        part = torch.empty(((N * OH * OW + 63) // 64, pc.Cout, 2), device=x.device, dtype=torch.float32)
    variant = ctypes.c_int(0) if (colsum or TRACE_CONV_VARIANT[0]) else None
    vref = ctypes.byref(variant) if variant is not None else None
    if x.dtype == torch.bfloat16:
        assert in_ab is None, 'the bf16 kernel does not fuse the producer GroupNorm (materialise with gn_apply)'
        if res_mask or colsum:
            assert res_mask and colsum and residual is not None and residual.dtype == torch.bfloat16 and not relu and not gn_part
            slots = conv2d_bf16_mask_slots(x.shape, pc, odt)
            assert slots > 0, 'this shape has no mask-mode instance (ask conv2d_bf16_mask_slots first)'
            part = torch.empty((slots, pc.Cout, 2), device=x.device, dtype=torch.float32)
            _lib.call('cpr_conv2d_fwd_bf16', _ptr(x), _ptr(pc.w), _ptr(pc.frag_image()), _ptr(out), _ptr(scale), _ptr(bias), _ptr(residual),
                      _ptr(part), N, H, W, Cin, pc.Cout, pc.KH, pc.KW, pc.stride, pc.padding, pc.Kpad, 2,
                      int(odt == torch.float32), vref, _stream())
            if variant is not None:
                TRACE_CONV_VARIANT[1] = ('bf16', variant.value)
            return out, TilePartials(part, slots, pc.Cout)
        _lib.call('cpr_conv2d_fwd_bf16', _ptr(x), _ptr(pc.w), _ptr(pc.frag_image()), _ptr(out), _ptr(scale), _ptr(bias), _ptr(residual),
                  _ptr(part), N, H, W, Cin, pc.Cout, pc.KH, pc.KW, pc.stride, pc.padding, pc.Kpad, int(relu),
                  int(odt == torch.float32), vref, _stream())
        if variant is not None:
            TRACE_CONV_VARIANT[1] = ('bf16', variant.value)
        return (out, part) if gn_part else out
    a = b = None
    if in_ab is not None:
        a, b = in_ab
    flags = (CONV_RELU if relu else 0) | (CONV_OUT_BF16 if odt == torch.bfloat16 else 0) | \
        (CONV_RES_MASK if res_mask else 0) | (CONV_COLSUM if colsum else 0)
    _lib.call('cpr_conv2d_fwd', _ptr(x), _ptr(pc.w), _ptr(out), _ptr(scale), _ptr(bias),
              _ptr(residual), _ptr(a), _ptr(b), _ptr(part), N, H, W, Cin, pc.Cout, pc.KH, pc.KW, pc.stride,
              pc.padding, pc.Kpad, flags, int(in_relu), vref, _stream())
    if variant is not None:
        TRACE_CONV_VARIANT[1] = ('fp32', variant.value)
    if colsum:
        bm = variant.value // 1000000
        return out, TilePartials(part, (N * OH * OW + bm - 1) // bm, pc.Cout)
    return (out, part) if gn_part else out


def conv2d_bf16_mask_slots(x_shape, pc, out_dtype=torch.bfloat16, fused_add=False):
    N, H, W, Cin = x_shape
    if pc.groups > 1 or (fused_add and (not WFRAG[0] or pc.Cout % 256 != 0)):
        return 0
    return _lib.call('cpr_conv2d_bf16_mask_slots', N, H, W, Cin, pc.Cout, pc.KH, pc.KW, pc.stride, pc.padding,
                     2 if fused_add else int(out_dtype == torch.float32), positive=True)


def conv2d_dgrad_bf16_fused(g16, pc, mask, add):
    _check(g16, ACT)
    pack_ready(pc)
    N, H, W, Cin = g16.shape
    OH, OW = pc.out_hw(H, W)
    shape = (N, OH, OW, pc.Cout)
    assert g16.dtype == torch.bfloat16 and pc.dtype == torch.bfloat16 and Cin == pc.Cin
    assert mask.dtype == torch.bfloat16 and add.dtype == torch.float32 and tuple(mask.shape) == shape and tuple(add.shape) == shape
    assert mask.is_contiguous() and add.is_contiguous()
    slots = conv2d_bf16_mask_slots(g16.shape, pc, fused_add=True)
    assert slots > 0, 'this shape has no fused instance (ask conv2d_bf16_mask_slots(..., fused_add=True) first)'
    out32 = torch.empty(shape, device=g16.device, dtype=torch.float32)
    out16 = torch.empty(shape, device=g16.device, dtype=torch.bfloat16)
    part = torch.empty((slots, pc.Cout, 2), device=g16.device, dtype=torch.float32)
    variant = ctypes.c_int(0) if TRACE_CONV_VARIANT[0] else None
    _lib.call('cpr_conv2d_dgrad_bf16_fused', _ptr(g16), _ptr(pc.w), _ptr(pc.frag_image()), _ptr(out32), _ptr(out16), _ptr(add), _ptr(mask),
              _ptr(part), N, H, W, Cin, pc.Cout, pc.KH, pc.KW, pc.stride, pc.padding, pc.Kpad,
              ctypes.byref(variant) if variant is not None else None, _stream())
    if variant is not None:
        TRACE_CONV_VARIANT[1] = ('bf16', variant.value)
    return out32, out16, TilePartials(part, slots, pc.Cout)


def conv1x1_stream(x, pc, scale=None, bias=None, residual=None, relu=False, res_mask=False):
    N, H, W, Cin = x.shape
    assert pc.KH == 1 and pc.stride == 1 and pc.padding == 0 and pc.Kpad == Cin and x.dtype == torch.float32
    out = torch.empty((N, H, W, pc.Cout), device=x.device, dtype=torch.float32)
    flags = (CONV_RELU if relu else 0) | (CONV_RES_MASK if res_mask else 0)
    _lib.call('cpr_conv1x1_stream_fwd', _ptr(x), _ptr(pc.w), _ptr(out), _ptr(scale), _ptr(bias), _ptr(residual),
              N * H * W, Cin, pc.Cout, flags, _stream())
    return out


def conv2d_dual(x, pc, x2, pc2, scale=None, bias=None, scale2=None, bias2=None, relu=False, out=None):
    _check(x, ACT)
    _check(x2, ACT)
    pack_ready(pc)
    pack_ready(pc2)
    N, H, W, Cin = x.shape
    N2, H2, W2, Cin2 = x2.shape
    assert x.dtype == torch.float32 and x2.dtype == torch.float32 and pc.dtype == torch.float32 and pc2.dtype == torch.float32
    assert N == N2 and Cin == pc.Cin and Cin2 == pc2.Cin and pc.Cout == pc2.Cout and pc2.KH == 1 and pc2.KW == 1 and pc2.padding == 0
    OH, OW = pc.out_hw(H, W)
    assert (OH, OW) == pc2.out_hw(H2, W2), 'the two sources must produce the same output grid'
    if out is None:
        out = torch.empty((N, OH, OW, pc.Cout), device=x.device, dtype=torch.float32)
    variant = ctypes.c_int(0) if TRACE_CONV_VARIANT[0] else None
    _lib.call('cpr_conv2d_dual_fwd', _ptr(x), _ptr(pc.w), _ptr(x2), _ptr(pc2.w), _ptr(out), _ptr(scale), _ptr(bias),
              _ptr(scale2), _ptr(bias2), N, H, W, Cin, pc.Cout, pc.KH, pc.KW, pc.stride, pc.padding, pc.Kpad, H2, W2, Cin2,
              pc2.stride, pc2.Kpad, CONV_RELU if relu else 0, ctypes.byref(variant) if variant is not None else None, _stream())
    if variant is not None:
        TRACE_CONV_VARIANT[1] = ('fp32', variant.value)
    return out


class TilePartials:

    def __init__(self, part, tiles, C):
        self.part, self.tiles, self.C = part, tiles, C

    def record_stream(self, stream):
        self.part.record_stream(stream)

    def reduce(self):
        cs = torch.empty((self.C,), device=self.part.device, dtype=torch.float32)
        ws = torch.empty((64 * self.C,), device=self.part.device, dtype=torch.float32)
        _lib.call('cpr_part_colsum', _ptr(self.part), _ptr(cs), _ptr(ws), self.tiles, self.C, _stream())
        return cs


def _sfx(x):
    return '_bf16' if x.dtype == torch.bfloat16 else ''


def bn_fold(gamma, beta, mean, var, eps, want_inv_sigma=False):
    C = gamma.numel()
    dev = gamma.device
    scale = torch.empty((C,), device=dev, dtype=torch.float32)
    shift = torch.empty((C,), device=dev, dtype=torch.float32)
    inv = torch.empty((C,), device=dev, dtype=torch.float32) if want_inv_sigma else None
    _lib.call('cpr_bn_fold', _ptr(_check(gamma.detach())), _ptr(_check(beta.detach())), _ptr(_check(mean)), _ptr(_check(var)),
              float(eps), _ptr(scale), _ptr(shift), _ptr(inv), C, _stream())
    return scale, shift, inv


def _bn_rows(y):
    C = y.shape[-1]
    M = y.numel() // C
    if M <= 1:
        raise ValueError('Expected more than 1 value per channel when training, got input size %s' % (tuple(y.shape),))
    assert C % 64 == 0, 'training-mode BatchNorm needs C % 64 == 0, got %d' % C
    return M, C


def _bn_vec(t, C):
    if t is None:
        return None
    t = _check(t.detach())
    assert t.numel() == C, 'per-channel vector of %d elements, want %d' % (t.numel(), C)
    return t


BnStats = collections.namedtuple('BnStats', 'mean rstd scale shift center cmean cshift')


def bn_batch_stats(y, gamma, beta, running_mean=None, running_var=None, num_batches_tracked=None, momentum=0.1, eps=1e-5, group=None):
    if sync_world_size(group) > 1:
        rec, _ = bn_sync_local_stats(y)
        return bn_sync_merge_stats(_sync_gather(rec, group), y, gamma, beta, running_mean, running_var, num_batches_tracked, momentum, eps)
    M, C = _bn_rows(_check(y))
    dev = y.device
    st = torch.empty((7, C), device=dev, dtype=torch.float32)
    ws = torch.empty((_lib.call('cpr_bn_train_ws', M, C, positive=True),), device=dev, dtype=torch.float32)
    if momentum is None:
        assert num_batches_tracked is not None, 'momentum None averages over num_batches_tracked'
    assert (running_mean is None) == (running_var is None), 'running_mean and running_var go together'
    bufs = [t for t in (running_mean, running_var) if t is not None]
    for t in bufs:
        _bn_vec(t, C)
    if num_batches_tracked is not None:
        assert _check(num_batches_tracked, torch.int64).numel() == 1
    _lib.call('cpr_bn_batch_stats', _ptr(y), _ptr(_bn_vec(gamma, C)), _ptr(_bn_vec(beta, C)), _ptr(running_mean),
              _ptr(running_var), _ptr(num_batches_tracked), -1.0 if momentum is None else float(momentum), float(eps),
              _ptr(st[0]), _ptr(st[1]), _ptr(st[2]), _ptr(st[3]), _ptr(st[4]), _ptr(st[5]), _ptr(st[6]), _ptr(ws), M, C, _stream())
    from torch.autograd.graph import increment_version
    for t in bufs + ([num_batches_tracked] if num_batches_tracked is not None else []):
        increment_version(t)
    return BnStats(*st.unbind(0))


def bn_apply(y, scale, shift, residual=None, relu=False, center=None, y2=None, scale2=None, shift2=None, center2=None, out=None):
    M, C = y.numel() // _check(y).shape[-1], y.shape[-1]
    for t in (residual, y2):
        if t is not None:
            assert _check(t).shape == y.shape, (t.shape, y.shape)
    assert residual is None or y2 is None
    assert y2 is not None or (scale2 is None and shift2 is None and center2 is None), 'scale2 / shift2 / center2 belong to y2'
    assert y2 is None or (scale2 is not None and shift2 is not None), 'the two-input form needs scale2 and shift2'
    if out is None:
        out = torch.empty_like(y)
    assert _check(out).shape == y.shape
    _lib.call('cpr_bn_apply', _ptr(y), _ptr(_bn_vec(center, C)), _ptr(_bn_vec(scale, C)), _ptr(_bn_vec(shift, C)), _ptr(residual),
              _ptr(y2), _ptr(_bn_vec(center2, C)), _ptr(_bn_vec(scale2, C)), _ptr(_bn_vec(shift2, C)), _ptr(out), M, C, int(relu),
              _stream())
    return out


def bn_train_bwd(dout, y, mean, rstd, gamma, mask=None, out_dgamma=None, out_dbeta=None, center=None, group=None, count=None):
    if sync_world_size(group) > 1:
        assert count is not None, 'the synchronised backward divides by the global row count of the forward (BnSyncStats.count)'
        rec, ws, dg, db = bn_sync_local_bwd(dout, y, mean, rstd, mask=mask, out_dgamma=out_dgamma, out_dbeta=out_dbeta, center=center)
        return bn_sync_merge_bwd(_sync_gather(rec, group), ws, count, dout, y, mean, rstd, gamma, mask=mask, center=center), dg, db
    M, C = _bn_rows(_check(y))
    assert _check(dout).shape == y.shape and (mask is None or _check(mask).shape == y.shape)
    dev = y.device
    dg = out_dgamma if out_dgamma is not None else torch.empty((C,), device=dev, dtype=torch.float32)
    db = out_dbeta if out_dbeta is not None else torch.empty((C,), device=dev, dtype=torch.float32)
    dy = torch.empty_like(y)
    ws = torch.empty((_lib.call('cpr_bn_train_ws', M, C, positive=True),), device=dev, dtype=torch.float32)
    _lib.call('cpr_bn_train_bwd', _ptr(dout), _ptr(mask), _ptr(y), _ptr(_bn_vec(center, C)), _ptr(_bn_vec(mean, C)), _ptr(_bn_vec(rstd, C)),
              _ptr(_bn_vec(gamma, C)), _ptr(dy), _ptr(_bn_vec(dg, C)), _ptr(_bn_vec(db, C)), _ptr(ws), M, C, _stream())
    return dy, dg, db


class BnSyncStats(BnStats):
    count = None


def sync_world_size(group=None):
    if group is None:
        return 1
    import torch.distributed as dist
    if not (dist.is_available() and dist.is_initialized()):
        return 1
    return dist.get_world_size(group)


def _sync_gather(record, group):
    import torch.distributed as dist
    R = dist.get_world_size(group)
# ... 1709 lines not shown
```

Measured before the change: 888.2.

## Split Winograd conv tail tiles across two workgroups by output-channel half

Adds a HALF template form to both Winograd conv kernels in which each workgroup computes only one 32-channel half of the 64-wide output block. For the 64 kernel, the wave-quantization remainder of tiles is launched as a second half-form launch. For wino32, small grids use the half form for all tiles. The aim is to fill idle CUs on small or tail-heavy grids. The cost is duplicated input-transform work, an extra launch, and more index bookkeeping.

```diff
diff --git a/include/cpr_hip.h b/include/cpr_hip.h
--- a/include/cpr_hip.h
+++ b/include/cpr_hip.h
@@ -36,6 +36,8 @@
 
 #define CPR_WINO_IN_B8 1
 #define CPR_WINO_OUT_B8 2
+#define CPR_WINO_FORM_FULL 8
+#define CPR_WINO_FORM_HALF 16
 int cpr_wino_pack_weights(const float* wgt, float* u, int Cin, int Cout, int Kpad, void* stream);
 int cpr_conv3x3_wino_fwd(const float* in, const float* u, float* out, const float* scale, const float* bias,
                          const float* in_a, const float* in_b, float* gn_part, int N, int H, int W, int Cin, int Cout,
diff --git a/pointtinybenchmark_amd/csrc/common.h b/pointtinybenchmark_amd/csrc/common.h
--- a/pointtinybenchmark_amd/csrc/common.h
+++ b/pointtinybenchmark_amd/csrc/common.h
@@ -13,6 +13,8 @@
 
 #define CPR_WINO_IN_B8 1
 #define CPR_WINO_OUT_B8 2
+#define CPR_WINO_FORM_FULL 8
+#define CPR_WINO_FORM_HALF 16
 
 #define CPR_CHECK_ARG(cond) \
     do {                    \
diff --git a/pointtinybenchmark_amd/csrc/conv_wino.hip b/pointtinybenchmark_amd/csrc/conv_wino.hip
--- a/pointtinybenchmark_amd/csrc/conv_wino.hip
+++ b/pointtinybenchmark_amd/csrc/conv_wino.hip
@@ -33,6 +33,7 @@
     int in_relu, out_b8;
     int N, H, W, Cin, Cout, relu, RY, RX, regions, tilesN, nch;
     int tpx;
+    int vb0, vb_end;
 };
 
 constexpr int WBUF = 16 * 64 * 8;
@@ -65,7 +66,7 @@
     }
 }
 
-template <int ABL, bool INB8, bool XF, int TSPREAD = 1, int VAR = 0>
+template <int ABL, bool INB8, bool XF, int TSPREAD = 1, int VAR = 0, bool HALF = false>
 __global__ __launch_bounds__(512, 1) void conv_wino_kernel(WinoParams p) {
     constexpr bool DEEP = (VAR & 1) != 0, UDMA = (VAR & 4) != 0, USINGLE = (VAR & 2) != 0 && !UDMA;
     constexpr int XFMAX = 512;
@@ -107,6 +108,7 @@
 
     struct Tile {
         int rg, tn, n, oy0, ox0, n0;
+        int hs;
         int voffA[2];
         unsigned uok;
         bool any_pad, valid;
@@ -117,6 +119,12 @@
     const int per_r = p.tpx > 0 ? (p.regions * ngrp + 7) / 8 : 0;
     auto setup = [&](int vb) {
         Tile t;
+        t.hs = 0;
+        if (HALF) {
+            const int s = vb >> 3;
+            t.hs = s & 1;
+            vb = p.vb0 + (s >> 1) * 8 + (vb & 7);
+        }
         if (p.tpx > 0) {
             const int x = vb & 7, s = vb >> 3;
             const int sr = s / p.tpx;
@@ -126,7 +134,7 @@
             if (!t.valid) { t.rg = 0; t.tn = 0; }
         } else {
             const int tile = (vb & 7) * per + (vb >> 3);
-            t.valid = vb < per * 8 && tile < T;
+            t.valid = vb < per * 8 && tile < T && vb < p.vb_end;
             const int tl = t.valid ? tile : 0;
             t.rg = tl / p.tilesN; t.tn = tl - t.rg * p.tilesN;
         }
@@ -273,6 +281,7 @@
     const int l31 = lane & 31, half = lane >> 5;
     const float* a_lds = Vs + (wi * 4 * 64 + l31) * 8 + 4 * (half ^ ((l31 >> 3) & 1));
     const float* b_lds = Us + (wi * 4 * 64 + nh * 32 + l31) * 8 + 4 * (half ^ ((l31 >> 3) & 1));
+    const float* const a_src = HALF ? a_lds + nh * 256 : a_lds;
     using Set0 = std::integral_constant<int, 0>;
     using Set1 = std::integral_constant<int, 1>;
 
@@ -283,6 +292,8 @@
     }
     for (int vb = blockIdx.x; cur.valid; vb += gridDim.x) {
     const int rg = cur.rg, n = cur.n, oy0 = cur.oy0, ox0 = cur.ox0, n0 = cur.n0;
+    const int hs = cur.hs;
+    const float* const b_src = HALF ? Us + (wi * 4 * 64 + hs * 32 + l31) * 8 + 4 * (half ^ ((l31 >> 3) & 1)) : b_lds;
 
     f32x16 acc[4][2];
 #pragma unroll
@@ -295,11 +306,11 @@
     f32x4 fa0[2], fb0, fa1[2], fb1;
 #define WFRAG(FA, FB, buf, j, z)                                                                                    \
     do {                                                                                                            \
-        if ((z) < 2) FA[(z) < 2 ? (z) : 0] = *reinterpret_cast<const f32x4*>(a_lds + (buf) * WBUF + (j) * 512 + ((z) < 2 ? (z) : 0) * 256); \
-        else FB = *reinterpret_cast<const f32x4*>(b_lds + (buf) * WBUF + (j) * 512);                                \
+        if ((z) < 2) { if (!HALF || (z) == 0) FA[(z) < 2 ? (z) : 0] = *reinterpret_cast<const f32x4*>(a_src + (buf) * WBUF + (j) * 512 + ((z) < 2 ? (z) : 0) * 256); } \
+        else FB = *reinterpret_cast<const f32x4*>(b_src + (buf) * WBUF + (j) * 512);                                \
     } while (0)
 #define WMFMA(FA, FB, j, q) \
-    acc[j][(q) & 1] = __builtin_amdgcn_mfma_f32_32x32x2f32(FA[(q) & 1][(q) >> 1], FB[(q) >> 1], acc[j][(q) & 1], 0, 0, 0)
+    do { if (!HALF || !((q) & 1)) acc[j][(q) & 1] = __builtin_amdgcn_mfma_f32_32x32x2f32(FA[(q) & 1][(q) >> 1], FB[(q) >> 1], acc[j][(q) & 1], 0, 0, 0); } while (0)
     r_a_pro(0, 0); r_a_pro(0, 1);
     r_a_pro(1, 0); r_a_pro(1, 1);
     if (UDMA) {
@@ -418,13 +429,14 @@
     __syncthreads();
     float* Rs = smem;
 #pragma unroll
-    for (int tb = 0; tb < 2; ++tb)
+    for (int tb = 0; tb < (HALF ? 1 : 2); ++tb)
 #pragma unroll
         for (int r = 0; r < 16; ++r) {
-            const int trow = tb * 32 + (r & 3) + 8 * (r >> 2) + 4 * half;
+            const int trow = (HALF ? nh : tb) * 32 + (r & 3) + 8 * (r >> 2) + 4 * half;
+            const int rcol = (HALF ? hs : nh) * 32 + l31;
             const float m0 = acc[0][tb][r], m1 = acc[1][tb][r], m2 = acc[2][tb][r], m3 = acc[3][tb][r];
-            Rs[((wi * 2 + 0) * 64 + trow) * 64 + nh * 32 + l31] = m0 + m1 + m2;
-            Rs[((wi * 2 + 1) * 64 + trow) * 64 + nh * 32 + l31] = m1 - m2 - m3;
+            Rs[((wi * 2 + 0) * 64 + trow) * 64 + rcol] = m0 + m1 + m2;
+            Rs[((wi * 2 + 1) * 64 + trow) * 64 + rcol] = m1 - m2 - m3;
         }
     __syncthreads();
     const int c4 = tid & 15;
@@ -435,8 +447,10 @@
     const __amdgpu_buffer_rsrc_t rs_out = __builtin_amdgcn_make_buffer_rsrc(
         p.out, 0, (int)((size_t)p.N * p.H * p.W * p.Cout * 4), 0x00020000);
     f32x4 gs = {0.f, 0.f, 0.f, 0.f}, gq = {0.f, 0.f, 0.f, 0.f};
+    const int klim = (HALF && (c4 >> 3) != hs) ? 0 : 2;
 #pragma unroll
     for (int k = 0; k < 2; ++k) {
+        if (HALF && k >= klim) break;
         const int t = (tid >> 4) + 32 * k;
         const int oy = oy0 + 2 * (t & 7), ox = ox0 + 2 * (t >> 3);
 #pragma unroll
@@ -474,7 +488,7 @@
             }
         }
         __syncthreads();
-        if (tid < 64) {
+        if (tid < 64 && (!HALF || (tid >> 5) == hs)) {
             float s = 0.f, q = 0.f;
 #pragma unroll
             for (int w8 = 0; w8 < 8; ++w8) { s += smem[(w8 * 64 + tid) * 2]; q += smem[(w8 * 64 + tid) * 2 + 1]; }
@@ -510,6 +524,7 @@
 constexpr int wino_sched = 0, wino_ablate = 0, wino_var = -1, wino_tpx = -1;
 #endif
 constexpr int WINO_VAR_DEFAULT = 4, WINO_TPX_DEFAULT = 0;
+constexpr int WINO_HALF_PCT = 65;
 extern "C" int cpr_wino_pack_weights(const float* wgt, float* u, int Cin, int Cout, int Kpad, hipStream_t stream) {
     CPR_CHECK_ARG(wgt && u && Cin > 0 && Cout > 0 && Cin % 8 == 0 && Cout % 64 == 0 && Kpad >= 9 * Cin);
     hipLaunchKernelGGL(wino_pack_kernel, dim3(cdiv(Cin * Cout, 256)), dim3(256), 0, stream, wgt, u, Cin, Cout, Kpad);
@@ -520,7 +535,8 @@
                            int Cout, int flags, int in_relu, int layout, hipStream_t stream) {
     CPR_CHECK_ARG(in && u && out && N > 0 && H > 0 && W > 0);
     CPR_CHECK_ARG(Cin > 0 && Cout > 0 && Cin % 16 == 0 && Cout % 64 == 0 && Cin >= 32);
-    CPR_CHECK_ARG((flags & ~CPR_CONV_RELU) == 0 && (layout & ~3) == 0);
+    CPR_CHECK_ARG((flags & ~CPR_CONV_RELU) == 0 && (layout & ~(CPR_WINO_IN_B8 | CPR_WINO_OUT_B8 | CPR_WINO_FORM_FULL | CPR_WINO_FORM_HALF)) == 0);
+    CPR_CHECK_ARG(!((layout & CPR_WINO_FORM_FULL) && (layout & CPR_WINO_FORM_HALF)));
     if (in_a) CPR_CHECK_ARG(in_b && Cin <= 512);
     if ((long long)N * H * W * Cin * 4 >= (1ll << 31) || (long long)N * H * W * Cout * 4 >= (1ll << 31)) return CPR_ERR_UNSUPPORTED;
     WinoParams p;
@@ -552,14 +568,28 @@
         if (vbs < grid) grid = (int)vbs;
     }
     const int var = wino_var >= 0 ? wino_var : WINO_VAR_DEFAULT;
-#define WLAUNCHV(A_, F_, V_)                                                                                                      \
+    const long long ids = p.tpx > 0 ? 0 : (T + 7) / 8 * 8;
+    long long full_ids = ids;
+    if (ids > 0 && T < (1ll << 29) && !(layout & CPR_WINO_FORM_FULL) && wino_var < 0 && wino_tpx < 0 && !wino_sched && !wino_ablate) {
+        const long long rem = ids % ncu;
+        if (layout & CPR_WINO_FORM_HALF) full_ids = 0;
+        else if (rem > 0 && (2 * rem + ncu - 1) / ncu * WINO_HALF_PCT < 100) full_ids = ids - rem;
+    }
+    p.vb0 = 0; p.vb_end = (int)(p.tpx > 0 ? 0 : full_ids);
+    WinoParams ph = p;
+    ph.vb0 = (int)full_ids; ph.vb_end = (int)ids;
+    int gridh = (int)(2 * (ids - full_ids) < ncu ? 2 * (ids - full_ids) : ncu);
+    if (full_ids < grid && p.tpx == 0) grid = (int)full_ids;
+#define WLAUNCHH(A_, F_, V_, H_, G_, P_)                                                                                          \
     do {                                                                                                                         \
         constexpr int TX_ = F_ == 2 ? 2 : 0 ^ F_, TP_ = F_ == 2 ? 2 : 1 ^ F_;                                                     \
-        if (b8 && xf) hipLaunchKernelGGL((conv_wino_kernel<A_, true, true, TX_, V_>), dim3(grid), dim3(512), 0, stream, p);       \
-        else if (b8) hipLaunchKernelGGL((conv_wino_kernel<A_, true, false, TP_, V_>), dim3(grid), dim3(512), 0, stream, p);       \
-        else if (xf) hipLaunchKernelGGL((conv_wino_kernel<A_, false, true, TX_, V_>), dim3(grid), dim3(512), 0, stream, p);       \
-        else hipLaunchKernelGGL((conv_wino_kernel<A_, false, false, TP_, V_>), dim3(grid), dim3(512), 0, stream, p);              \
+        if (G_ <= 0) break;                                                                                                      \
+        if (b8 && xf) hipLaunchKernelGGL((conv_wino_kernel<A_, true, true, TX_, V_, H_>), dim3(G_), dim3(512), 0, stream, P_);    \
+        else if (b8) hipLaunchKernelGGL((conv_wino_kernel<A_, true, false, TP_, V_, H_>), dim3(G_), dim3(512), 0, stream, P_);    \
+        else if (xf) hipLaunchKernelGGL((conv_wino_kernel<A_, false, true, TX_, V_, H_>), dim3(G_), dim3(512), 0, stream, P_);    \
+        else hipLaunchKernelGGL((conv_wino_kernel<A_, false, false, TP_, V_, H_>), dim3(G_), dim3(512), 0, stream, P_);           \
     } while (0)
+#define WLAUNCHV(A_, F_, V_) WLAUNCHH(A_, F_, V_, false, grid, p)
 #define WLAUNCH(A_, F_) WLAUNCHV(A_, F_, WINO_VAR_DEFAULT)
 #ifdef CPR_BENCH_HOOKS
     if ((var != WINO_VAR_DEFAULT || wino_sched == 2) && !wino_ablate) {
@@ -592,9 +622,13 @@
         }
     } else
 #endif
-    WLAUNCH(0, 0);
+    {
+        WLAUNCH(0, 0);
+        WLAUNCHH(0, 0, WINO_VAR_DEFAULT, true, gridh, ph);
+    }
 #undef WLAUNCH
 #undef WLAUNCHV
+#undef WLAUNCHH
     CPR_LAUNCH_STATUS();
 }
 
diff --git a/pointtinybenchmark_amd/csrc/conv_wino32.hip b/pointtinybenchmark_amd/csrc/conv_wino32.hip
--- a/pointtinybenchmark_amd/csrc/conv_wino32.hip
+++ b/pointtinybenchmark_amd/csrc/conv_wino32.hip
@@ -51,7 +51,7 @@
     }
 }
 
-template <bool XF, int ABL = 0>
+template <bool XF, int ABL = 0, bool HALF = false>
 __global__ __launch_bounds__(256, 2) void conv_wino32_kernel(Wino32Params p) {
     __shared__ __attribute__((aligned(16))) float smem[W32_LDS];
     float* Vs = smem;
@@ -88,7 +88,8 @@
     }
 
     int cur_n = -1;
-    for (int vb = blockIdx.x;; vb += gridDim.x) {
+    const int hs = HALF ? ((int)blockIdx.x >> 3) & 1 : 0;
+    for (int vb = HALF ? ((int)blockIdx.x >> 4) * 8 + ((int)blockIdx.x & 7) : (int)blockIdx.x;; vb += gridDim.x >> (HALF ? 1 : 0)) {
         const int tile = (vb & 7) * per + (vb >> 3);
         if (!(vb < per * 8 && tile < T)) break;
         const int rg = tile / p.tilesN, tn = tile - rg * p.tilesN;
@@ -189,11 +190,11 @@
             dma_u(c + 2, (c + 2) % 3);
             dma_a(c + 4, c & 3);
             const float* va = Vs + b * W32_V + a_rd;
-            const float* ub = Us + uslot * W32_U + b_rd;
+            const float* ub = Us + uslot * W32_U + b_rd + (HALF ? hs * 128 : 0);
             f32x2 fa[2], fb[2][2];
             fa[0] = *reinterpret_cast<const f32x2*>(va);
             fb[0][0] = *reinterpret_cast<const f32x2*>(ub);
-            fb[0][1] = *reinterpret_cast<const f32x2*>(ub + 128);
+            if (!HALF) fb[0][1] = *reinterpret_cast<const f32x2*>(ub + 128);
 #pragma unroll
             for (int j = 0; j < 4; ++j) {
                 const int cu = j & 1, nx = cu ^ 1;
@@ -201,10 +202,10 @@
                 if (j < 3 && !(ABL & 8)) {
                     fa[nx] = *reinterpret_cast<const f32x2*>(va + (j + 1) * 128);
                     fb[nx][0] = *reinterpret_cast<const f32x2*>(ub + (j + 1) * 256);
-                    fb[nx][1] = *reinterpret_cast<const f32x2*>(ub + (j + 1) * 256 + 128);
+                    if (!HALF) fb[nx][1] = *reinterpret_cast<const f32x2*>(ub + (j + 1) * 256 + 128);
                 }
                 __builtin_amdgcn_sched_barrier(0);
-                acc[j][1] = __builtin_amdgcn_mfma_f32_32x32x2f32(fa[cu].x, fb[cu][1].x, acc[j][1], 0, 0, 0);
+                if (!HALF) acc[j][1] = __builtin_amdgcn_mfma_f32_32x32x2f32(fa[cu].x, fb[cu][1].x, acc[j][1], 0, 0, 0);
                 if (j == 0) { t_read((c + 1) & 3, 0); }
                 if (j == 1) { t_read((c + 1) & 3, 1); }
                 if (j == 2) { t_read((c + 1) & 3, 2); }
@@ -212,7 +213,7 @@
                 acc[j][0] = __builtin_amdgcn_mfma_f32_32x32x2f32(fa[cu].y, fb[cu][0].y, acc[j][0], 0, 0, 0);
                 if (j == 1) affine_pass(c + 2, (c + 2) & 3);
                 __builtin_amdgcn_sched_barrier(0);
-                acc[j][1] = __builtin_amdgcn_mfma_f32_32x32x2f32(fa[cu].y, fb[cu][1].y, acc[j][1], 0, 0, 0);
+                if (!HALF) acc[j][1] = __builtin_amdgcn_mfma_f32_32x32x2f32(fa[cu].y, fb[cu][1].y, acc[j][1], 0, 0, 0);
                 if (j == 3) t_write(b ^ 1);
                 __builtin_amdgcn_sched_barrier(0);
             }
@@ -227,13 +228,14 @@
 
         float* Rs = smem;
 #pragma unroll
-        for (int nb = 0; nb < 2; ++nb)
+        for (int nb = 0; nb < (HALF ? 1 : 2); ++nb)
 #pragma unroll
             for (int r = 0; r < 16; ++r) {
                 const int trow = (r & 3) + 8 * (r >> 2) + 4 * half;
+                const int rcol = (HALF ? hs : nb) * 32 + l31;
                 const float m0 = acc[0][nb][r], m1 = acc[1][nb][r], m2 = acc[2][nb][r], m3 = acc[3][nb][r];
-                Rs[((wave * 2 + 0) * 32 + trow) * 64 + nb * 32 + l31] = m0 + m1 + m2;
-                Rs[((wave * 2 + 1) * 32 + trow) * 64 + nb * 32 + l31] = m1 - m2 - m3;
+                Rs[((wave * 2 + 0) * 32 + trow) * 64 + rcol] = m0 + m1 + m2;
+                Rs[((wave * 2 + 1) * 32 + trow) * 64 + rcol] = m1 - m2 - m3;
             }
         __syncthreads();
         const int c4 = tid & 15;
@@ -244,8 +246,10 @@
         const __amdgpu_buffer_rsrc_t rs_out = __builtin_amdgcn_make_buffer_rsrc(
             p.out, 0, (int)((size_t)p.N * p.H * p.W * p.Cout * 4), 0x00020000);
         f32x4 gs = {0.f, 0.f, 0.f, 0.f}, gq = {0.f, 0.f, 0.f, 0.f};
+        const bool c4_live = !HALF || (c4 >> 3) == hs;
 #pragma unroll
         for (int k = 0; k < 4; ++k) {
+            if (!c4_live) break;
             const int it = (tid >> 4) + 16 * k;
             const int t = it & 31, bq = it >> 5;
             const int oy = oy0 + 2 * (t >> 3), ox = ox0 + 2 * (t & 7) + bq;
@@ -281,7 +285,7 @@
                 }
             }
             __syncthreads();
-            if (tid < 64) {
+            if (tid < 64 && (!HALF || (tid >> 5) == hs)) {
                 float s = 0.f, q = 0.f;
 #pragma unroll
                 for (int w4 = 0; w4 < 4; ++w4) { s += smem[(w4 * 64 + tid) * 2]; q += smem[(w4 * 64 + tid) * 2 + 1]; }
@@ -303,6 +307,7 @@
 #else
 constexpr int w32_ablate = 0, w32_wg_per_cu = 2, w32_stagger_pct = 100;
 #endif
+constexpr int W32_HALF_MAX_PCT = 50;
 extern "C" int cpr_wino32_pack_weights(const float* wgt, float* u, int Cin, int Cout, int Kpad, hipStream_t stream) {
     CPR_CHECK_ARG(wgt && u && Cin > 0 && Cout > 0 && Cin % 4 == 0 && Cout % 64 == 0 && Kpad >= 9 * Cin);
     hipLaunchKernelGGL(wino32_pack_kernel, dim3(cdiv(Cin * Cout, 256)), dim3(256), 0, stream, wgt, u, Cin, Cout, Kpad);
@@ -316,7 +321,8 @@
                              int Cout, int flags, int in_relu, int layout, hipStream_t stream) {
     CPR_CHECK_ARG(in && u && out && N > 0 && H > 0 && W > 0);
     CPR_CHECK_ARG(Cin > 0 && Cout > 0 && Cin % 8 == 0 && Cout % 64 == 0 && Cin >= 16);
-    CPR_CHECK_ARG((flags & ~CPR_CONV_RELU) == 0 && (layout & ~3) == 0);
+    CPR_CHECK_ARG((flags & ~CPR_CONV_RELU) == 0 && (layout & ~(CPR_WINO_IN_B8 | CPR_WINO_OUT_B8 | CPR_WINO_FORM_FULL | CPR_WINO_FORM_HALF)) == 0);
+    CPR_CHECK_ARG(!((layout & CPR_WINO_FORM_FULL) && (layout & CPR_WINO_FORM_HALF)));
     if (in_a) CPR_CHECK_ARG(in_b && Cin <= W32_XFMAX);
     if ((long long)N * H * W * Cin * 4 >= (1ll << 31) || (long long)N * H * W * Cout * 4 >= (1ll << 31)) return CPR_ERR_UNSUPPORTED;
     Wino32Params p;
@@ -339,16 +345,24 @@
     }
     ncu = (ncu + 7) / 8 * 8;
     int grid = (int)((T + 7) / 8 * 8);
+    const long long ids = grid;
+    bool half_form = (layout & CPR_WINO_FORM_HALF) != 0;
+    if (!(layout & (CPR_WINO_FORM_FULL | CPR_WINO_FORM_HALF)) && !w32_ablate) half_form = ids * 100 <= (long long)ncu * W32_HALF_MAX_PCT;
+    if (T >= (1ll << 29)) half_form = false;
+    if (half_form) grid *= 2;
     if (grid > w32_wg_per_cu * ncu) grid = w32_wg_per_cu * ncu;
-    p.stagger = grid > ncu ? (int)(((long long)p.nch * 16 * 65 * w32_stagger_pct / 100 + 8127) / 8128) : 0;
+    if (half_form) grid = grid / 16 * 16;
+    p.stagger = grid > ncu ? (int)(((long long)p.nch * (half_form ? 8 : 16) * 65 * w32_stagger_pct / 100 + 8127) / 8128) : 0;
+#define W32LH(A_, H_)                                                                                                 \
+    do {                                                                                                              \
+        if (in_a) hipLaunchKernelGGL((conv_wino32_kernel<true, A_, H_>), dim3(grid), dim3(256), 0, stream, p);       \
+        else hipLaunchKernelGGL((conv_wino32_kernel<false, A_, H_>), dim3(grid), dim3(256), 0, stream, p);           \
+    } while (0)
+#define W32L(A_) W32LH(A_, false)
 #ifdef CPR_BENCH_HOOKS
-#define W32L(A_)                                                                                                      \
-    do {                                                                                                              \
-        if (in_a) hipLaunchKernelGGL((conv_wino32_kernel<true, A_>), dim3(grid), dim3(256), 0, stream, p);           \
-        else hipLaunchKernelGGL((conv_wino32_kernel<false, A_>), dim3(grid), dim3(256), 0, stream, p);               \
-    } while (0)
+    if (half_form && w32_ablate) return CPR_ERR_UNSUPPORTED;
     switch (w32_ablate) {
-        case 0: W32L(0); break;
+        case 0: if (half_form) W32LH(0, true); else W32L(0); break;
         case 1: W32L(1); break;
         case 2: W32L(2); break;
         case 3: W32L(3); break;
@@ -358,11 +372,11 @@
         case 15: W32L(15); break;
         default: return CPR_ERR_UNSUPPORTED;
     }
+#else
+    if (half_form) W32LH(0, true); else W32L(0);
+#endif
 #undef W32L
-#else
-    if (in_a) hipLaunchKernelGGL((conv_wino32_kernel<true>), dim3(grid), dim3(256), 0, stream, p);
-    else hipLaunchKernelGGL((conv_wino32_kernel<false>), dim3(grid), dim3(256), 0, stream, p);
-#endif
+#undef W32LH
     CPR_LAUNCH_STATUS();
 }
 
diff --git a/pointtinybenchmark_amd/ops.py b/pointtinybenchmark_amd/ops.py
--- a/pointtinybenchmark_amd/ops.py
+++ b/pointtinybenchmark_amd/ops.py
@@ -301,6 +301,9 @@
 
 WINO_TILE = ['auto']
 
+WINO_FORM = ['auto']
+_WINO_FORM_BITS = {'auto': 0, 'full': 8, 'half': 16}
+
 
 def wino_instance(pc, H, W, fused_affine):
     can32 = pc.Cin % 8 == 0 and (not fused_affine or pc.Cin <= 256)
@@ -360,7 +363,7 @@
         assert Cin <= 512
     _lib.call('cpr_conv3x3_wino32_fwd' if inst == '32' else 'cpr_conv3x3_wino_fwd', _ptr(x), _ptr(getattr(pc, attr)), _ptr(out),
               _ptr(scale), _ptr(bias), _ptr(a), _ptr(b), _ptr(part), N, H, W, Cin, pc.Cout, CONV_RELU if relu else 0, int(in_relu),
-              (1 if in_b8 else 0) | (2 if out_b8 else 0), _stream())
+              (1 if in_b8 else 0) | (2 if out_b8 else 0) | _WINO_FORM_BITS[WINO_FORM[0]], _stream())
     if TRACE_CONV_VARIANT[0]:
         TRACE_CONV_VARIANT[1] = ('wino32' if inst == '32' else 'wino',
                                  (1 if in_b8 else 0) | (2 if out_b8 else 0) | (4 if in_ab is not None else 0))
```

Result: no change. 887.7 (-0.1%).
